# gongaa/video-layout-generation

Measured on AMD Instinct MI355X. Metric: training clips/sec at (B,T,N)=(32,16,64) d=256; 1/2/4/8-GPU scaling, higher is better.
Workload: dtype f32

## Files before the change

include/vlg_hip.h:

```cpp
#ifndef VLG_HIP_H
#define VLG_HIP_H

#include <stdint.h>

typedef uint16_t vlg_bf16;

#ifdef __cplusplus
extern "C" {
#endif

#define VLG_ERR_SHAPE   1001
#define VLG_ERR_ALIGN   1002

int         vlg_abi_version(void);
const char* vlg_build_arch(void);

#ifdef VLG_DIAG
void vlg_debug_set_clock_probe(unsigned long long* buf);
void vlg_debug_set_conv_probe(unsigned long long* buf);
void vlg_debug_set_gemm_bk(int bk);
void vlg_debug_set_gemm_run(int run);
#endif

int vlg_embed_fwd(const int64_t* slot_class, const float* slot_box,
                  const float* cls_emb, const float* box_w, const float* box_b,
                  const float* time_emb, float* x,
                  int B, int T, int N, int d, int vocab, void* stream);
int vlg_embed_bwd_slabs(void);
int vlg_embed_bwd_slabs_for(int B, int T, int N, int d, int vocab);
int vlg_embed_bwd(const float* dx, const int64_t* slot_class, const float* slot_box,
                  float* slabs, int64_t slab_stride, int64_t slab_capacity,
                  int B, int T, int N, int d, int vocab, void* stream);

int vlg_layernorm_fwd(const float* x, const float* gamma, const float* beta,
                      float* y, float* mean, float* rstd,
                      int64_t rows, int d, float eps, void* stream);
int vlg_layernorm_fwd_bf16(const float* x, const float* gamma, const float* beta,
                           vlg_bf16* y, float* mean, float* rstd,
                           int64_t rows, int d, float eps, void* stream);
int vlg_layernorm_bwd_slabs(int64_t rows);
int vlg_layernorm_bwd(const float* dy, const float* x, const float* mean, const float* rstd,
                      const float* gamma, const float* dres, float* dx_out,
                      float* slabs, int64_t slab_stride, int64_t slab_capacity,
                      int64_t rows, int d, void* stream);
int vlg_layernorm_bwd_bf16(const vlg_bf16* dy, const float* x, const float* mean, const float* rstd,
                           const float* gamma, const float* dres, float* dx_out,
                           float* slabs, int64_t slab_stride, int64_t slab_capacity,
                           int64_t rows, int d, void* stream);

#define VLG_EPI_NONE   0
#define VLG_EPI_BIAS   1
#define VLG_EPI_GELU   2
#define VLG_EPI_RESID  4
#define VLG_EPI_DGELU  8
#define VLG_EPI_BF16   16
#define VLG_EPI_SPLIT3 256
#define VLG_EPI_ACT_GELU 512
#define VLG_EPI_GELU_GRAD 1024
#define VLG_EPI_MUL    2048
#define VLG_EPI_A_BF16   32
#define VLG_EPI_B_BF16   64
#define VLG_EPI_OUT_BF16 128
int vlg_linear_fwd(const void* A, int lda, const void* W, int ldw, const float* bias,
                   void* C, int ldc, const void* aux_in, void* aux_out,
                   int64_t M, int N, int K, int epilogue, void* stream);
int vlg_linear_dgrad(const void* dY, int ldy, const void* W, int ldw,
                     void* dX, int ldx, const void* aux_in,
                     int64_t M, int N, int K, int epilogue, void* stream);
int vlg_linear_wgrad_slabs(int64_t M, int N, int K);
int vlg_linear_wgrad_slabs_for(int64_t M, int N, int K, int flags);
int vlg_linear_wgrad(const void* dY, int ldy, const void* X, int ldx,
                     float* slabs, int64_t slab_stride, int64_t slab_capacity,
                     int64_t M, int N, int K, int flags , void* stream);
int vlg_linear_dgrad_wgrad(const void* dY, int ldy, const void* W, int ldw, void* dX, int ldx, const void* aux_in,
                           const void* X, int ldxx, float* slabs, int64_t slab_stride, int64_t slab_capacity,
                           int64_t M, int N, int K, int epilogue,
                           const int64_t* rider_table , int rider_rows, void* stream);
#define VLG_CALL_FWD   0
#define VLG_CALL_DGRAD 1
#define VLG_CALL_WGRAD 2
#define VLG_CALL_PAIR  3
#define VLG_GEMM_F32   0
#define VLG_GEMM_BF16  1
#define VLG_GEMM_F32X3 2
typedef struct vlg_gemm_problem {
    int bm, bn, bk;
    int run;
    int splits;
    int blocks;
    int64_t rows_per_split;
} vlg_gemm_problem;
typedef struct vlg_gemm_plan {
    int family;
    int launches;
    int problems;
    int fused;
    vlg_gemm_problem p[2];
} vlg_gemm_plan;
int vlg_linear_plan(int call, int64_t M, int N, int K, int flags, int lda, int ldb, int ldc, int ldxx, vlg_gemm_plan* plan);


int vlg_attention_fwd(const float* qkv, float* o, int64_t n_seq, int T, int d, void* stream);
int vlg_attention_bwd(const float* qkv, const float* dout, float* dqkv,
                      int64_t n_seq, int T, int d, void* stream);
int vlg_attention_fwd_bf16(const vlg_bf16* qkv, vlg_bf16* o, int64_t n_seq, int T, int d, void* stream);
int vlg_attention_bwd_bf16(const vlg_bf16* qkv, const vlg_bf16* dout, vlg_bf16* dqkv,
                           int64_t n_seq, int T, int d, void* stream);

int vlg_layout_loss_scratch(void);
int vlg_layout_loss(const float* out, int ld, const int64_t* tgt_class, const float* tgt_box,
                    const float* valid, float* dout, float* loss_out, float* scratch,
                    int B, int T, int N, int n_classes, float beta, float iou_eps,
                    float w_reg, float w_iou, float w_ce, void* stream);

int vlg_attention_clip_fwd(const float* qkv, const float* valid, float* out, float* lse,
                           int64_t B, int T, int N, int d, void* stream);
int vlg_attention_clip_bwd(const float* qkv, const float* valid, const float* out, const float* dout, const float* lse,
                           float* delta, float* dqkv, int64_t B, int T, int N, int d, void* stream);
int vlg_attention_clip_fwd_bf16(const vlg_bf16* qkv, const float* valid, vlg_bf16* out, float* lse,
                                int64_t B, int T, int N, int d, void* stream);
int vlg_attention_clip_bwd_bf16(const vlg_bf16* qkv, const float* valid, const vlg_bf16* out, const vlg_bf16* dout,
                                const float* lse, float* delta, vlg_bf16* dqkv,
                                int64_t B, int T, int N, int d, void* stream);

int vlg_reduce_slabs(const float* slabs, int64_t slab_stride, int n_slabs,
                     float* dst, int64_t len, void* stream);

int vlg_adam_step_graph(float* param, const float* grad, float* exp_avg, float* exp_avg_sq, vlg_bf16* shadow,
                        int64_t n, float* state, int advance, float lr, float beta1, float beta2, float eps,
                        float grad_scale, void* stream);

int vlg_reduce_slabs_table(const int64_t* table, int n_rows, int blocks_per_row, void* stream);
int vlg_sum_partials_table(const int64_t* table, int n_rows, void* stream);

int vlg_adam_step(float* param, const float* grad, float* exp_avg, float* exp_avg_sq,
                  int64_t n, int step, float lr, float beta1, float beta2, float eps,
                  float grad_scale, void* stream);
int vlg_adam_step_bf16(float* param, const float* grad, float* exp_avg, float* exp_avg_sq, vlg_bf16* shadow,
                       int64_t n, int step, float lr, float beta1, float beta2, float eps,
                       float grad_scale, void* stream);

int vlg_image_loss_scratch(void);
int vlg_ce_nchw(const float* logits, const int64_t* target, float* dlogits, float* loss,
                float* scratch, int b, int C, int64_t hw, float grad_scale, void* stream);
int vlg_l1_mean(const float* a, const float* b, float* da, float* loss, float* scratch,
                int64_t n, float grad_scale, void* stream);
int vlg_gradient_loss(const float* a, const float* b, float* da, float* loss, float* scratch,
                      int planes, int H, int W, float grad_scale, void* stream);
int vlg_ssim_loss(const float* x, const float* y, float* dx, float* loss, float* scratch,
                  int b, int C, int H, int W, float grad_scale, void* stream);
int vlg_affine_nchw(const float* src, float* dst, int b, int C, int64_t hw, const float* shift_host,
                    const float* scale_host, void* stream);
int vlg_prep_input(const float* e1, const float* seg1, const float* frame1,
                   const float* frame2, const float* seg2, const float* e2,
                   const float* frame3, const int64_t* seg3,
                   float* x10, float* frame3_out, int64_t* seg3_out,
                   int b, int H, int W, int flip, void* stream);

int vlg_argmax_nchw(const float* logits, float* out, int b, int C, int64_t hw, void* stream);
int vlg_rollout_input(const float* e_a, const float* seg_a, const float* img_a, const float* img_b,
                      const float* seg_b, const float* e_b, float* x10, int b, int64_t hw, void* stream);

#define VLG_CEPI_BIAS   1
#define VLG_CEPI_RESID  2
#define VLG_CEPI_PRELU  4
#define VLG_CEPI_DPRELU 8
#define VLG_CEPI_ACCUM  16
#define VLG_CEPI_CIN4   32
int vlg_conv3x3_fwd(const float* in, const float* w, const float* bias, float* out, const float* resid,
                    const float* rowmask, const float* prelu_slope, const int* rowtab, int64_t rows_out,
                    int cin_p, int cout, int cout_p, int wp_in, int act_ch, int epilogue,
                    float* workspace ,
                    int64_t workspace_capacity , void* stream);
int vlg_conv3x3_fwd_splits(int64_t rows_out, int cin_p, int cout, int cout_p);
int64_t vlg_conv3x3_fwd_workspace(int64_t rows_out, int cin_p, int cout, int cout_p);
int vlg_conv3x3_dgrad_slabs(int64_t rows_in, int cin_p);
int vlg_conv3x3_dgrad(const float* dout, const float* w, float* din, const float* x_in,
                      const float* rowmask_in, const float* prelu_slope, float* da_slab,
                      const int* tap_tables, int64_t tab_stride, int64_t rows_in, int cin_p, int cout_p,
                      int wp, int act_ch, int epilogue,
                      float* workspace ,
                      int64_t workspace_capacity ,
                      int da_capacity , void* stream);
int vlg_conv3x3_dgrad_splits(int64_t rows_in, int cin_p, int cout_p);
int64_t vlg_conv3x3_dgrad_workspace(int64_t rows_in, int cin_p, int cout_p);
int vlg_conv3x3_wgrad_slabs(int64_t rows, int cin_p, int cout_p);
int vlg_conv3x3_wgrad(const float* dout, const float* in, float* slabs, int64_t slab_stride, int64_t slab_capacity,
                      const int* rowtab, const float* prelu_slope, int64_t rows, int cin_p, int cout_p,
                      int wp_in, int act_ch, void* stream);
int vlg_conv3x3_fwd_bf16(const float* in, const float* w, const float* bias, float* out, const float* resid,
                         const float* rowmask, const float* prelu_slope, const int* rowtab, int64_t rows_out,
                         int cin_p, int cout, int cout_p, int wp_in, int act_ch, int epilogue, float* workspace,
                         int64_t workspace_capacity, void* stream);
int vlg_conv3x3_fwd_bf16_splits(int64_t rows_out, int cin_p, int cout, int cout_p);
int64_t vlg_conv3x3_fwd_bf16_workspace(int64_t rows_out, int cin_p, int cout, int cout_p);
int vlg_conv3x3_dgrad_bf16_slabs(int64_t rows_in, int cin_p);
int vlg_conv3x3_dgrad_bf16(const float* dout, const float* w, float* din, const float* x_in,
                           const float* rowmask_in, const float* prelu_slope, float* da_slab,
                           const int* tap_tables, int64_t tab_stride, int64_t rows_in, int cin_p, int cout_p,
                           int wp, int act_ch, int epilogue, float* workspace, int64_t workspace_capacity,
                           int da_capacity, void* stream);
int vlg_conv3x3_dgrad_bf16_splits(int64_t rows_in, int cin_p, int cout_p);
int64_t vlg_conv3x3_dgrad_bf16_workspace(int64_t rows_in, int cin_p, int cout_p);
int vlg_conv3x3_wgrad_bf16_slabs(int64_t rows, int cin_p, int cout_p);
int vlg_conv3x3_wgrad_bf16(const float* dout, const float* in, float* slabs, int64_t slab_stride, int64_t slab_capacity,
                           const int* rowtab, const float* prelu_slope, int64_t rows, int cin_p, int cout_p,
                           int wp_in, int act_ch, void* stream);
int vlg_nchw_to_padded(const float* src, float* dst, int b, int C, int H, int W, int cp, int coord_c0, void* stream);
int vlg_padded_to_nchw(const float* src, float* dst, int b, int C, int H, int W, int cp, void* stream);
int vlg_fill_coords(float* dst, int b, int H, int W, int cp, int coord_c0, void* stream);
int vlg_upsample2x_fwd(const float* in, float* out, int b, int h, int w, int cp, void* stream);
int vlg_upsample2x_bwd(const float* dout, float* din, int b, int h, int w, int cp, int accumulate, void* stream);
int vlg_maxpool2x2(const float* in, float* out, int b, int h, int w, int cp, void* stream);
int vlg_score1x1_relu(const float* in, const float* w, const float* bias, float* out, int b, int H, int W,
                      int C, int cp, void* stream);
int vlg_hed_head(const float* s0, const float* s1, const float* s2, const float* s3, const float* s4,
                 const float* combine_w, const float* combine_b, float* out , int b, int H, int W,
                 void* stream);
int vlg_maxpool2x2_bwd(const float* in, const float* dout, float* din, int b, int h, int w, int cp, void* stream);
int vlg_l1_relu_padded(const float* a, const float* b, float* da, float* loss, float* scratch ,
                       int64_t rows, int cp, int64_t count, float grad_scale, void* stream);
int vlg_add_rows(float* dst, const float* src, int64_t n, int accumulate, void* stream);
int vlg_sum_partials(const float* partials, int n, float* dst, int accumulate, void* stream);

#ifdef __cplusplus
}
#endif
#endif
```

video-layout-generation_amd/csrc/layernorm.hip:

```cpp
#include "common.h"

#define LN_BLOCK 256
#define LN_WAVES (LN_BLOCK / 64)
#define LN_BWD_MAX_BLOCKS 512

template <int E, bool V4>
struct RowIO {
    template <typename EL>
    __device__ static __forceinline__ void load(const EL* __restrict__ row, int lane, float (&v)[E]) {
        if constexpr (V4) {
#pragma unroll
            for (int i = 0; i < E / 4; ++i) {
                const float4 t = ld4(row + 4 * lane + 256 * i);
                v[4 * i] = t.x; v[4 * i + 1] = t.y; v[4 * i + 2] = t.z; v[4 * i + 3] = t.w;
            }
        } else {
#pragma unroll
            for (int i = 0; i < E; ++i) v[i] = ld1(row + lane + 64 * i);
        }
    }
    template <typename EL>
    __device__ static __forceinline__ void store(EL* __restrict__ row, int lane, const float (&v)[E]) {
        if constexpr (V4) {
#pragma unroll
            for (int i = 0; i < E / 4; ++i)
                st4(row + 4 * lane + 256 * i, make_float4(v[4 * i], v[4 * i + 1], v[4 * i + 2], v[4 * i + 3]));
        } else {
#pragma unroll
            for (int i = 0; i < E; ++i) st1(row + lane + 64 * i, v[i]);
        }
    }
    __device__ static __forceinline__ int col(int lane, int j) {
        if constexpr (V4) return 4 * lane + 256 * (j >> 2) + (j & 3);
        else return lane + 64 * j;
    }
};

#define LN_ROWS(E) ((E) <= 4 ? 4 : (E) <= 8 ? 2 : 1)

template <int E, bool V4, typename EY = float>
__global__ __launch_bounds__(LN_BLOCK) void ln_fwd_kernel(
    const float* __restrict__ x, const float* __restrict__ gamma, const float* __restrict__ beta,
    EY* __restrict__ y, float* __restrict__ mean, float* __restrict__ rstd, int64_t rows, float eps) {
    constexpr int d = E * 64, R = LN_ROWS(E);
    const int lane = threadIdx.x & 63;
    const int64_t wave = (int64_t)blockIdx.x * LN_WAVES + (threadIdx.x >> 6);
    const int64_t nwaves = (int64_t)gridDim.x * LN_WAVES;
    float g[E], b[E];
    RowIO<E, V4>::load(gamma, lane, g);
    RowIO<E, V4>::load(beta, lane, b);
    for (int64_t r0 = wave * R; r0 < rows; r0 += nwaves * R) {
        float v[R][E];
#pragma unroll
        for (int i = 0; i < R; ++i) {
            const int64_t r = r0 + i < rows ? r0 + i : rows - 1;
            RowIO<E, V4>::load(x + r * d, lane, v[i]);
        }
#pragma unroll
        for (int i = 0; i < R; ++i) {
            float s = 0.f;
#pragma unroll
            for (int j = 0; j < E; ++j) s += v[i][j];
            const float mu = wave_sum(s) * (1.0f / d);
            float q = 0.f;
#pragma unroll
            for (int j = 0; j < E; ++j) { const float t = v[i][j] - mu; q += t * t; }
            const float rs = 1.0f / sqrtf(wave_sum(q) * (1.0f / d) + eps);
#pragma unroll
            for (int j = 0; j < E; ++j) v[i][j] = (v[i][j] - mu) * rs * g[j] + b[j];
            if (r0 + i < rows) {
                RowIO<E, V4>::store(y + (r0 + i) * d, lane, v[i]);
                if (lane == 0) { mean[r0 + i] = mu; rstd[r0 + i] = rs; }
            }
        }
    }
}

template <int E, bool V4, typename EY = float>
__global__ __launch_bounds__(LN_BLOCK) void ln_bwd_kernel(
    const EY* __restrict__ dy, const float* __restrict__ x, const float* __restrict__ mean,
    const float* __restrict__ rstd, const float* __restrict__ gamma, const float* __restrict__ dres,
    float* __restrict__ dx_out, float* __restrict__ slabs, int64_t slab_stride, int64_t rows) {
    constexpr int d = E * 64, R = LN_ROWS(E);
    __shared__ float red[LN_WAVES][2 * d];
    const int lane = threadIdx.x & 63, w = threadIdx.x >> 6;
    const int64_t wave = (int64_t)blockIdx.x * LN_WAVES + w;
    const int64_t nwaves = (int64_t)gridDim.x * LN_WAVES;
    float g[E], dg[E], db[E];
    RowIO<E, V4>::load(gamma, lane, g);
#pragma unroll
    for (int j = 0; j < E; ++j) { dg[j] = 0.f; db[j] = 0.f; }
    for (int64_t r0 = wave * R; r0 < rows; r0 += nwaves * R) {
        float gy[R][E], xv[R][E], o[R][E], mu[R], rs[R];
#pragma unroll
        for (int i = 0; i < R; ++i) {
            const int64_t r = r0 + i < rows ? r0 + i : rows - 1;
            RowIO<E, V4>::load(dy + r * d, lane, gy[i]);
            RowIO<E, V4>::load(x + r * d, lane, xv[i]);
            if (dres != nullptr) RowIO<E, V4>::load(dres + r * d, lane, o[i]);
            else {
#pragma unroll
                for (int j = 0; j < E; ++j) o[i][j] = 0.f;
            }
            mu[i] = mean[r];
            rs[i] = rstd[r];
        }
#pragma unroll
        for (int i = 0; i < R; ++i) {
            const float live = r0 + i < rows ? 1.f : 0.f;
            float s1 = 0.f, s2 = 0.f;
#pragma unroll
            for (int j = 0; j < E; ++j) {
                const float xh = (xv[i][j] - mu[i]) * rs[i];
                const float gl = gy[i][j] * live;
                const float a = gy[i][j] * g[j];
                dg[j] += gl * xh;
                db[j] += gl;
                s1 += a;
                s2 += a * xh;
                xv[i][j] = xh;
                gy[i][j] = a;
            }
            s1 = wave_sum(s1) * (1.0f / d);
            s2 = wave_sum(s2) * (1.0f / d);
#pragma unroll
            for (int j = 0; j < E; ++j) o[i][j] += rs[i] * (gy[i][j] - s1 - xv[i][j] * s2);
            if (r0 + i < rows) RowIO<E, V4>::store(dx_out + (r0 + i) * d, lane, o[i]);
        }
    }
#pragma unroll
    for (int j = 0; j < E; ++j) {
        const int c = RowIO<E, V4>::col(lane, j);
        red[w][c] = dg[j];
        red[w][d + c] = db[j];
    }
    __syncthreads();
    float* slab = slabs + (int64_t)blockIdx.x * slab_stride;
    for (int c = threadIdx.x; c < 2 * d; c += LN_BLOCK) {
        float s = 0.f;
#pragma unroll
        for (int k = 0; k < LN_WAVES; ++k) s += red[k][c];
        slab[c] = s;
    }
}

static int ln_fwd_blocks(int64_t rows) {
    int64_t b = (rows + LN_WAVES - 1) / LN_WAVES;
    return (int)(b > 2048 ? 2048 : (b < 1 ? 1 : b));
}
static int ln_bwd_blocks(int64_t rows) {
    int64_t b = (rows + LN_WAVES - 1) / LN_WAVES;
    return (int)(b > LN_BWD_MAX_BLOCKS ? LN_BWD_MAX_BLOCKS : (b < 1 ? 1 : b));
}

#define LN_DISPATCH(d, CALL)                                 \
    switch (d) {                                             \
        case 64:   { CALL(1, false) } break;                 \
        case 128:  { CALL(2, false) } break;                 \
        case 192:  { CALL(3, false) } break;                 \
        case 256:  { CALL(4, true) } break;                  \
        case 512:  { CALL(8, true) } break;                  \
        case 768:  { CALL(12, true) } break;                 \
        case 1024: { CALL(16, true) } break;                 \
        default: return VLG_ERR_SHAPE;                       \
    }

extern "C" int vlg_layernorm_fwd(const float* x, const float* gamma, const float* beta, float* y,
                                 float* mean, float* rstd, int64_t rows, int d, float eps, void* stream) {
    if (rows < 1) return VLG_ERR_SHAPE;
    if (!vlg_aligned16(x) || !vlg_aligned16(y) || !vlg_aligned16(gamma) || !vlg_aligned16(beta)) return VLG_ERR_ALIGN;
    const dim3 grid(ln_fwd_blocks(rows)), block(LN_BLOCK);
    hipStream_t s = (hipStream_t)stream;
#define CALL(E, V4) hipLaunchKernelGGL((ln_fwd_kernel<E, V4>), grid, block, 0, s, x, gamma, beta, y, mean, rstd, rows, eps);
    LN_DISPATCH(d, CALL)
#undef CALL
    return vlg_last_error();
}

extern "C" int vlg_layernorm_bwd_slabs(int64_t rows) { return ln_bwd_blocks(rows); }

extern "C" int vlg_layernorm_bwd(const float* dy, const float* x, const float* mean, const float* rstd,
                                 const float* gamma, const float* dres, float* dx_out, float* slabs,
                                 int64_t slab_stride, int64_t slab_capacity, int64_t rows, int d, void* stream) {
    if (rows < 1 || slab_stride < 2 * (int64_t)d) return VLG_ERR_SHAPE;
    if (slab_capacity < (int64_t)ln_bwd_blocks(rows) * slab_stride) return VLG_ERR_SHAPE;
    if (!vlg_aligned16(dy) || !vlg_aligned16(x) || !vlg_aligned16(gamma) || !vlg_aligned16(dx_out) ||
        (dres && !vlg_aligned16(dres))) return VLG_ERR_ALIGN;
    const dim3 grid(ln_bwd_blocks(rows)), block(LN_BLOCK);
    hipStream_t s = (hipStream_t)stream;
#define CALL(E, V4) hipLaunchKernelGGL((ln_bwd_kernel<E, V4>), grid, block, 0, s, dy, x, mean, rstd, gamma, dres, dx_out, slabs, slab_stride, rows);
    LN_DISPATCH(d, CALL)
#undef CALL
    return vlg_last_error();
}

extern "C" int vlg_layernorm_fwd_bf16(const float* x, const float* gamma, const float* beta, vlg_bf16* y,
                                      float* mean, float* rstd, int64_t rows, int d, float eps, void* stream) {
    if (rows < 1) return VLG_ERR_SHAPE;
    if (!vlg_aligned16(x) || !vlg_aligned8(y) || !vlg_aligned16(gamma) || !vlg_aligned16(beta)) return VLG_ERR_ALIGN;
    const dim3 grid(ln_fwd_blocks(rows)), block(LN_BLOCK);
    hipStream_t s = (hipStream_t)stream;
    bf16_t* yb = reinterpret_cast<bf16_t*>(y);
#define CALL(E, V4) hipLaunchKernelGGL((ln_fwd_kernel<E, V4, bf16_t>), grid, block, 0, s, x, gamma, beta, yb, mean, rstd, rows, eps);
    LN_DISPATCH(d, CALL)
#undef CALL
    return vlg_last_error();
}

extern "C" int vlg_layernorm_bwd_bf16(const vlg_bf16* dy, const float* x, const float* mean, const float* rstd,
                                      const float* gamma, const float* dres, float* dx_out, float* slabs,
                                      int64_t slab_stride, int64_t slab_capacity, int64_t rows, int d, void* stream) {
    if (rows < 1 || slab_stride < 2 * (int64_t)d) return VLG_ERR_SHAPE;
    if (slab_capacity < (int64_t)ln_bwd_blocks(rows) * slab_stride) return VLG_ERR_SHAPE;
    if (!vlg_aligned8(dy) || !vlg_aligned16(x) || !vlg_aligned16(gamma) || !vlg_aligned16(dx_out) ||
        (dres && !vlg_aligned16(dres))) return VLG_ERR_ALIGN;
    const dim3 grid(ln_bwd_blocks(rows)), block(LN_BLOCK);
    hipStream_t s = (hipStream_t)stream;
    const bf16_t* dyb = reinterpret_cast<const bf16_t*>(dy);
#define CALL(E, V4) hipLaunchKernelGGL((ln_bwd_kernel<E, V4, bf16_t>), grid, block, 0, s, dyb, x, mean, rstd, gamma, dres, dx_out, slabs, slab_stride, rows);
    LN_DISPATCH(d, CALL)
#undef CALL
    return vlg_last_error();
}
```

video-layout-generation_amd/csrc/loss.hip:

```cpp
#include "common.h"

#define LOSS_BLOCK 256
#define LOSS_TOK 128
#define LOSS_ROWF 28
#define LOSS_MAX_BLOCKS 1024
#define NCLS 20
#define NOUT (NCLS + 4)
#define LOSS_F4 (NOUT / 4)
#define LOSS_NV (LOSS_TOK * LOSS_F4 / LOSS_BLOCK)

#define LOSS_SCRATCH (4 + 4 * LOSS_MAX_BLOCKS)

__global__ __launch_bounds__(LOSS_BLOCK) void layout_loss_kernel(
    const float* __restrict__ out, int ld, const int64_t* __restrict__ tgt_class,
    const float* __restrict__ tgt_box, const float* __restrict__ valid, float* __restrict__ dout,
    float* __restrict__ scratch, float* __restrict__ loss_out, int B, int T, int N, float beta, float iou_eps,
    float w_reg, float w_iou, float w_ce) {
    __shared__ __attribute__((aligned(16))) float rows[LOSS_TOK * LOSS_ROWF];
    __shared__ float red[LOSS_BLOCK / 64];
    __shared__ float cnt_sh;
    __shared__ int last_sh;
    const int64_t M = (int64_t)B * T * N;
    const int tid = threadIdx.x;
    float inv_cnt = 0.f;
    float s_reg = 0.f, s_iou = 0.f, s_ce = 0.f;
    for (int64_t m0 = (int64_t)blockIdx.x * LOSS_TOK; m0 < M; m0 += (int64_t)gridDim.x * LOSS_TOK) {
        float4 stage[LOSS_NV];
#pragma unroll
        for (int i = 0; i < LOSS_NV; ++i) {
            const int f = tid + i * LOSS_BLOCK, tok = f / LOSS_F4, c = f - tok * LOSS_F4;
            stage[i] = (m0 + tok < M) ? ld4(out + (m0 + tok) * ld + 4 * c) : f4_zero();
        }
        const int64_t m = m0 + tid;
        const bool mine = tid < LOSS_TOK && m < M;
        float w = 0.f;
        int64_t cls = 0;
        float4 tb = f4_zero();
        if (mine) {
            const int t = (int)(m % T);
            const int64_t bn = m / T;
            const int n = (int)(bn % N);
            const int64_t b = bn / N;
            const int64_t src = (b * T + t) * N + n;
            w = valid[src];
            cls = tgt_class[src];
            tb = ld4(tgt_box + src * 4);
        }
        if (m0 == (int64_t)blockIdx.x * LOSS_TOK) {
            float c = 0.f;
            const int64_t n4 = M >> 2;
            int64_t i = tid;
            for (; i + 15 * LOSS_BLOCK < n4; i += 16 * LOSS_BLOCK) {
                float4 v[16];
#pragma unroll
                for (int u = 0; u < 16; ++u) v[u] = ld4(valid + 4 * (i + u * LOSS_BLOCK));
#pragma unroll
                for (int u = 0; u < 16; ++u) c += (v[u].x + v[u].y) + (v[u].z + v[u].w);
            }
            for (; i < n4; i += LOSS_BLOCK) {
                const float4 v = ld4(valid + 4 * i);
                c += (v.x + v.y) + (v.z + v.w);
            }
            for (int64_t j = 4 * n4 + tid; j < M; j += LOSS_BLOCK) c += valid[j];
            c = block_sum(c, red);
            if (tid == 0) cnt_sh = 1.0f / fmaxf(c, 1.0f);
            __syncthreads();
            inv_cnt = cnt_sh;
        }
#pragma unroll
        for (int i = 0; i < LOSS_NV; ++i) {
            const int f = tid + i * LOSS_BLOCK, tok = f / LOSS_F4, c = f - tok * LOSS_F4;
            st4(rows + tok * LOSS_ROWF + 4 * c, stage[i]);
        }
        __syncthreads();
        if (mine) {
            float* row = rows + tid * LOSS_ROWF;
            float v[NOUT];
#pragma unroll
            for (int c = 0; c < LOSS_F4; ++c) {
                const float4 q = ld4(row + 4 * c);
                v[4 * c] = q.x; v[4 * c + 1] = q.y; v[4 * c + 2] = q.z; v[4 * c + 3] = q.w;
            }
            float g[NOUT];
            cls = cls < 0 ? 0 : (cls >= NCLS ? NCLS - 1 : cls);
            float mx = v[0];
#pragma unroll
            for (int c = 1; c < NCLS; ++c) mx = fmaxf(mx, v[c]);
            float se = 0.f, vt = 0.f;
#pragma unroll
            for (int c = 0; c < NCLS; ++c) {
                g[c] = expf(v[c] - mx);
                se += g[c];
                vt = (c == cls) ? v[c] : vt;
            }
            const float ce = logf(se) + mx - vt;
            const float gs = w * inv_cnt * w_ce / se;
#pragma unroll
            for (int c = 0; c < NCLS; ++c) g[c] = g[c] * gs - ((c == cls) ? w * inv_cnt * w_ce : 0.f);
            const float tg[4] = {tb.x, tb.y, tb.z, tb.w};
            float p[4], dp[4];
            float reg = 0.f;
#pragma unroll
            for (int k = 0; k < 4; ++k) {
                p[k] = 1.0f / (1.0f + expf(-v[NCLS + k]));
                const float df = p[k] - tg[k], ad = fabsf(df);
                const bool quad = ad < beta;
                reg += quad ? 0.5f * df * df / beta : ad - 0.5f * beta;
                dp[k] = (quad ? df / beta : (df > 0.f ? 1.f : (df < 0.f ? -1.f : 0.f))) * (w_reg * 0.25f);
            }
            const float ax1 = p[0] - 0.5f * p[2], ax2 = p[0] + 0.5f * p[2];
            const float ay1 = p[1] - 0.5f * p[3], ay2 = p[1] + 0.5f * p[3];
            const float bx1 = tg[0] - 0.5f * tg[2], bx2 = tg[0] + 0.5f * tg[2];
            const float by1 = tg[1] - 0.5f * tg[3], by2 = tg[1] + 0.5f * tg[3];
            const float iw_raw = fminf(ax2, bx2) - fmaxf(ax1, bx1);
            const float ih_raw = fminf(ay2, by2) - fmaxf(ay1, by1);
            const float iw = fmaxf(iw_raw, 0.f), ih = fmaxf(ih_raw, 0.f);
            const float inter = iw * ih;
            const float uni = p[2] * p[3] + tg[2] * tg[3] - inter;
            const float den = uni + iou_eps;
            const float iou = inter / den;
            const float di_dinter = (den + inter) / (den * den);
            const float di_darea = -inter / (den * den);
            const float x2s = (ax2 < bx2) ? 1.f : (ax2 == bx2 ? 0.5f : 0.f);
            const float x1s = (ax1 > bx1) ? 1.f : (ax1 == bx1 ? 0.5f : 0.f);
            const float y2s = (ay2 < by2) ? 1.f : (ay2 == by2 ? 0.5f : 0.f);
            const float y1s = (ay1 > by1) ? 1.f : (ay1 == by1 ? 0.5f : 0.f);
            const float diw = (iw_raw >= 0.f) ? ih * di_dinter : 0.f;
            const float dih = (ih_raw >= 0.f) ? iw * di_dinter : 0.f;
            float di[4];
            di[0] = diw * (x2s - x1s);
            di[1] = dih * (y2s - y1s);
            di[2] = diw * 0.5f * (x2s + x1s) + di_darea * p[3];
            di[3] = dih * 0.5f * (y2s + y1s) + di_darea * p[2];
#pragma unroll
            for (int k = 0; k < 4; ++k)
                g[NCLS + k] = (dp[k] - w_iou * di[k]) * p[k] * (1.f - p[k]) * w * inv_cnt;
#pragma unroll
            for (int c = 0; c < LOSS_F4; ++c)
                st4(row + 4 * c, make_float4(g[4 * c], g[4 * c + 1], g[4 * c + 2], g[4 * c + 3]));
            s_reg += w * reg * 0.25f;
            s_iou += w * (1.f - iou);
            s_ce += w * ce;
        }
        __syncthreads();
#pragma unroll
        for (int i = 0; i < LOSS_NV; ++i) {
            const int f = tid + i * LOSS_BLOCK, tok = f / LOSS_F4, c = f - tok * LOSS_F4;
            if (m0 + tok < M) st4(dout + (m0 + tok) * ld + 4 * c, ld4(rows + tok * LOSS_ROWF + 4 * c));
        }
        __syncthreads();
    }
    s_reg = block_sum(s_reg, red);
    s_iou = block_sum(s_iou, red);
    s_ce = block_sum(s_ce, red);
    if (tid == 0) {
        float* part = scratch + 4 + 4 * blockIdx.x;
        part[0] = s_reg * inv_cnt; part[1] = s_iou * inv_cnt; part[2] = s_ce * inv_cnt; part[3] = 0.f;
        __threadfence();
        int* ticket = reinterpret_cast<int*>(scratch) + 1;
        const int drawn = atomicAdd(ticket, 1);
        last_sh = (drawn == (int)gridDim.x - 1) ? 1 : 0;
    }
    __syncthreads();
    if (last_sh && tid < 64) {
        __threadfence();
        float a = 0.f, b = 0.f, c = 0.f;
        for (int i = tid; i < (int)gridDim.x; i += 64) {
            const float4 q = ld4(scratch + 4 + 4 * i);
            a += q.x; b += q.y; c += q.z;
        }
        a = wave_sum(a); b = wave_sum(b); c = wave_sum(c);
        if (tid == 0) {
            loss_out[0] = w_reg * a + w_iou * b + w_ce * c;
            loss_out[1] = a; loss_out[2] = b; loss_out[3] = c;
            *(reinterpret_cast<int*>(scratch) + 1) = 0;
        }
    }
}

extern "C" int vlg_layout_loss_scratch(void) { return LOSS_SCRATCH; }

extern "C" int vlg_layout_loss(const float* out, int ld, const int64_t* tgt_class, const float* tgt_box,
                               const float* valid, float* dout, float* loss_out, float* scratch, int B, int T,
                               int N, int n_classes, float beta, float iou_eps, float w_reg, float w_iou,
                               float w_ce, void* stream) {
    if (n_classes != NCLS || B < 1 || T < 1 || N < 1 || ld < NOUT || (ld & 3) || !(beta > 0.f)) return VLG_ERR_SHAPE;
    if (!vlg_aligned16(out) || !vlg_aligned16(dout) || !vlg_aligned16(tgt_box) || !vlg_aligned16(valid)) return VLG_ERR_ALIGN;
    const int64_t M = (int64_t)B * T * N;
    if (!loss_out || !scratch || !vlg_aligned16(scratch)) return VLG_ERR_ALIGN;
    int64_t blocks = (M + LOSS_TOK - 1) / LOSS_TOK;
    if (blocks > LOSS_MAX_BLOCKS) blocks = LOSS_MAX_BLOCKS;
    hipStream_t s = (hipStream_t)stream;
    hipLaunchKernelGGL(layout_loss_kernel, dim3((unsigned)blocks), dim3(LOSS_BLOCK), 0, s, out, ld, tgt_class,
                       tgt_box, valid, dout, scratch, loss_out, B, T, N, beta, iou_eps, w_reg, w_iou, w_ce);
    return vlg_last_error();
}
```

video-layout-generation_amd/vlg/engine.py:

```python
from __future__ import annotations

import math
import os
from typing import Dict, Optional

import torch

from . import hip
from .hip import (EPI_A_BF16, EPI_B_BF16, EPI_BIAS, EPI_DGELU, EPI_GELU, EPI_NONE, EPI_OUT_BF16, EPI_RESID,
                  call, ptr)
from .spec import (ADAM_BETA1, ADAM_BETA2, ADAM_EPS, ADAM_LR, BOX_DIM, IOU_EPS, LN_EPS, LOSS_W_CE,
                   LOSS_W_REG, LOSS_W_STRUCT, SMOOTH_L1_BETA, LayoutConfig, param_layout)


def init_params(cfg: LayoutConfig, seed: int) -> Dict[str, torch.Tensor]:
    layout, _ = param_layout(cfg)
    g = torch.Generator().manual_seed(seed)
    fan_in = {name[:-2] + "_b": shape[1] for name, (_, shape) in layout.items() if name.endswith("_w")}
    out: Dict[str, torch.Tensor] = {}
    for name, (_, shape) in layout.items():
        base = name.split(".")[-1]
        if base in ("cls_emb", "time_emb"):
            t = torch.randn(shape, generator=g, dtype=torch.float32)
        elif base.endswith("_g"):
            t = torch.ones(shape)
        elif base.startswith("ln") and base.endswith("_b"):
            t = torch.zeros(shape)
        elif base.endswith("_w"):
            t = (torch.rand(shape, generator=g, dtype=torch.float32) * 2 - 1) * (1.0 / math.sqrt(shape[1]))
        else:
            t = (torch.rand(shape, generator=g, dtype=torch.float32) * 2 - 1) * (1.0 / math.sqrt(fan_in[name]))
        out[name] = t
    return out


class LayoutEngine:

    def __init__(self, cfg: LayoutConfig, device: torch.device, seed: int = 1024,
                 lr: float = ADAM_LR, beta1: float = ADAM_BETA1, precision: str = "fp32", padded_slots: bool = True):
        cfg.validate()
        if precision not in ("fp32", "bf16", "bf16_mfma", "fp32x3"):
            raise ValueError("precision must be fp32, fp32x3, bf16 or bf16_mfma")
        self.padded_slots = bool(padded_slots)
        self._masked = self.padded_slots
        self.precision = precision
        self.gemm_flags = {"fp32": 0, "fp32x3": hip.EPI_SPLIT3}.get(precision, hip.EPI_BF16)
        self.bf16_store = precision == "bf16"
        self.gelu_grad_saved = precision in ("fp32", "bf16", "bf16_mfma") and os.environ.get("VLG_GELU_GRAD_SAVED", "1") != "0"
        self._epi_ff1 = EPI_BIAS | EPI_GELU | (hip.EPI_GELU_GRAD if self.gelu_grad_saved else 0)
        self._epi_dff2 = hip.EPI_MUL if self.gelu_grad_saved else EPI_DGELU
        self._sfx = "_bf16" if self.bf16_store else ""
        hip.load()
        if device.type != "cuda":
            raise hip.HipError("LayoutEngine needs a HIP device (got %s); there is no CPU path" % device)
        self.cfg, self.device = cfg, device
        self.lr, self.beta1 = float(lr), float(beta1)
        self.layout, self.n_params = param_layout(cfg)
        f32 = dict(dtype=torch.float32, device=device)
        self.params = torch.zeros(self.n_params, **f32)
        self.grads_ext = torch.zeros(self.n_params + 4, **f32)
        self.grads = self.grads_ext[:self.n_params]
        self.exp_avg = torch.zeros(self.n_params, **f32)
        self.exp_avg_sq = torch.zeros(self.n_params, **f32)
        self.step_count = 0
        self.adam_state = None
        self.params_bf16 = torch.zeros(self.n_params, dtype=torch.bfloat16, device=device) if self.bf16_store else None
        self.load_params(init_params(cfg, seed))
        self._alloc_workspace(cfg.tokens)
        self.loss_out = self.grads_ext[self.n_params:]
        self.timer = None

    def view(self, flat: torch.Tensor, name: str) -> torch.Tensor:
        off, shape = self.layout[name]
        return flat[off:off + math.prod(shape)].view(shape)

    def p(self, name: str) -> torch.Tensor:
        return self.view(self.params, name)

    def pw(self, name: str) -> torch.Tensor:
        return self.view(self.params_bf16 if self.bf16_store else self.params, name)

    def _sync_device_step(self) -> None:
        if self.adam_state is not None:
            self.adam_state.view(torch.int32)[2] = int(self.step_count)

    def _refresh_shadow(self) -> None:
        if self.params_bf16 is not None:
            self.params_bf16.copy_(self.params)

    def g(self, name: str) -> torch.Tensor:
        return self.view(self.grads, name)

    def load_params(self, tensors: Dict[str, torch.Tensor]) -> None:
        for name in self.layout:
            self.p(name).copy_(tensors[name].to(torch.float32))
        self._refresh_shadow()

    def named_params(self) -> Dict[str, torch.Tensor]:
        return {n: self.p(n) for n in self.layout}

    def named_grads(self) -> Dict[str, torch.Tensor]:
        return {n: self.g(n) for n in self.layout}

    def state_dict(self) -> Dict[str, object]:
        return {"params": self.params.detach().cpu().clone(), "exp_avg": self.exp_avg.cpu().clone(),
                "exp_avg_sq": self.exp_avg_sq.cpu().clone(), "step": self.step_count,
                "layout": {k: (o, tuple(s)) for k, (o, s) in self.layout.items()}}

    def load_state_dict(self, sd: Dict[str, object]) -> None:
        if tuple(sd["params"].shape) != (self.n_params,):
            raise ValueError("checkpoint has %d parameters, model has %d" % (sd["params"].numel(), self.n_params))
        self.params.copy_(sd["params"])
        self._refresh_shadow()
        self.exp_avg.copy_(sd["exp_avg"])
        self.exp_avg_sq.copy_(sd["exp_avg_sq"])
        self.step_count = int(sd["step"])
        self._sync_device_step()

    def optimizer_state(self) -> Dict[str, object]:
        return {"exp_avg": self.exp_avg.cpu().clone(), "exp_avg_sq": self.exp_avg_sq.cpu().clone(),
                "step": int(self.step_count), "lr": self.lr, "beta1": self.beta1}

    def load_optimizer(self, st: Dict[str, object]) -> None:
        if st["exp_avg"].numel() != self.n_params:
            raise ValueError("optimizer state has %d elements, model has %d" % (st["exp_avg"].numel(), self.n_params))
        self.exp_avg.copy_(st["exp_avg"])
        self.exp_avg_sq.copy_(st["exp_avg_sq"])
        self.step_count = int(st["step"])
        self._sync_device_step()

    def _alloc_workspace(self, tokens: int) -> None:
        cfg, d, ff = self.cfg, self.cfg.d, self.cfg.d_ff
        f32 = dict(dtype=torch.float32, device=self.device)
        M = self.capacity = tokens
        L = cfg.n_layers
        lib = hip.load()
        act = dict(dtype=torch.bfloat16 if self.bf16_store else torch.float32, device=self.device)
        self.x = torch.empty(L + 1, M, d, **f32)
        self.h1 = torch.empty(L, M, d, **act)
        self.qkv = torch.empty(L, M, 3 * d, **act)
        self.att = torch.empty(L, M, d, **act)
        self.xmid = torch.empty(L, M, d, **f32)
        self.h2 = torch.empty(L, M, d, **act)
        self.u = torch.empty(L, M, ff, **act)
        self.gl = torch.empty(L, M, ff, **act)
        self.stats = torch.empty(2 * L + 1, 2, M, **f32)
        self.xf = torch.empty(M, d, **act)
        self.out = torch.empty(M, cfg.n_out, **f32)
        self.dout = torch.empty(M, cfg.n_out, **f32)
        self.dx = torch.empty(M, d, **f32)
        self.dh = torch.empty(M, d, **act)
        self.du = torch.empty(M, ff, **act)
        self.dqkv = torch.empty(M, 3 * d, **act)
        self.loss_scratch = torch.zeros(lib.vlg_layout_loss_scratch(), **f32)
        if cfg.attention == "clip":
            self.lse = torch.empty(L, cfg.n_heads * M, **f32)
            self.delta = torch.empty(cfg.n_heads * M, **f32)
        emb_len = self.layout["l0.ln1_g"][0]
        need = [lib.vlg_embed_bwd_slabs() * emb_len, lib.vlg_layernorm_bwd_slabs(M) * 2 * d]
        for (n, k) in ((3 * d, d), (d, d), (ff, d), (d, ff), (cfg.n_out, d)):
            need.append(lib.vlg_linear_wgrad_slabs_for(M, n, k, self.gemm_flags) * (n * k + n))
        self.side = torch.cuda.Stream(device=self.device)
        self.overlap_wgrad = os.environ.get("VLG_OVERLAP_WGRAD", "0") == "1"
        self.group_reduce = not self.overlap_wgrad
        self.pair_backward = (not self.overlap_wgrad and self.precision in ("fp32", "bf16")
                              and os.environ.get("VLG_PAIR_BACKWARD", "1") == "1")
        self.ride_reduces = False
        if self.group_reduce:
            pad = lambda v: (v + 3) // 4 * 4
            layer = sum(pad(v) for v in need[2:6]) + 2 * pad(need[1])
            head = pad(need[6]) + pad(need[1])
            self.garenas = [torch.empty(max(layer, head, pad(need[0])), **f32) for _ in range(2)]
            self._gsel = 0
            self._goff = 0
            self._grows: list = []
            self._gtables: Dict[tuple, torch.Tensor] = {}
            self._pending = None
            self.ride_reduces = self.pair_backward and os.environ.get("VLG_RIDE_REDUCE", "1") == "1"
        else:
            self.slabs = torch.empty(max(need[:2]), **f32)
            self.slabs_w = torch.empty(max(need[2:]), **f32)

    @staticmethod
    def _stream() -> int:
        return torch.cuda.current_stream().cuda_stream

    def _arena(self, kind: str, need: int = 0) -> torch.Tensor:
        if self.group_reduce:
            garena = self.garenas[self._gsel]
            off = self._goff
            if off + need > garena.numel():
                raise RuntimeError("partial-sum arena of %d floats is too small for %d more" % (garena.numel(), need))
            self._goff = off + (need + 3) // 4 * 4
            self._gcur = garena.data_ptr() + 4 * off
            return garena[off:off + need]
        return self.slabs_w if kind == "w" else self.slabs

    def _reduce(self, kind: str, stride: int, n_slabs: int, dst_off: int, dst_len: int) -> None:
        dst = self.grads.data_ptr() + 4 * dst_off
        if self.group_reduce:
            self._grows.append((self._gcur, stride, n_slabs, dst, dst_len))
            return
        call("vlg_reduce_slabs", ptr(self.slabs_w if kind == "w" else self.slabs), stride, n_slabs, dst, dst_len, self._stream())

    def _table(self, rows: tuple) -> torch.Tensor:
        table = self._gtables.get(rows)
        if table is None:
            table = torch.tensor([v for row in rows for v in row], dtype=torch.int64, device=self.device)
            self._gtables[rows] = table
        return table

    def _join_reduces(self, defer: bool = False, then=None) -> None:
        if not self.group_reduce:
            if then is not None:
                then()
            return
        rows = tuple(self._grows)
        self._grows = []
        self._goff = 0
        if defer and self.ride_reduces and rows and self._pending is None:
            self._pending = (rows, then)
            self._gsel ^= 1
            return
        waiting, self._pending = self._pending, None
        if waiting is not None:
            rows = waiting[0] + rows
        if rows:
            call("vlg_reduce_slabs_table", ptr(self._table(rows)), len(rows), 128, self._stream())
        if waiting is not None and waiting[1] is not None:
            waiting[1]()
        if then is not None:
            then()

    def _take_rider(self):
        if not self.group_reduce or self._pending is None:
            self._rider_bytes = 0.0
            return 0, 0, None
        (rows, then), self._pending = self._pending, None
        self._rider_bytes = 4.0 * sum((n_slabs + 1) * length for (_, _, n_slabs, _, length) in rows)
        return ptr(self._table(rows)), len(rows), then

    def _timed(self, family: str, flops: float, name: str, *args, nbytes: float = 0.0) -> None:
        if self.timer is None or (self.timer.only is not None and family not in self.timer.only):
            call(name, *args)
        else:
            with self.timer.section(family, flops, nbytes):
                call(name, *args)

    @staticmethod
    def _storage_bits(a=None, b=None, out=None) -> int:
        bf = torch.bfloat16
        return ((EPI_A_BF16 if a is not None and a.dtype == bf else 0) | (EPI_B_BF16 if b is not None and b.dtype == bf else 0) |
                (EPI_OUT_BF16 if out is not None and out.dtype == bf else 0))

    def _linear(self, a, w, b, c, M, N, K, epi, aux_in=None, aux_out=None):
        nb = (a.element_size() * M * K + w.element_size() * N * K +
              c.element_size() * M * N * (1 + (aux_in is not None) + (aux_out is not None)))
        flags = epi | self.gemm_flags | self._storage_bits(a, w, c)
        self._timed("gemm_fwd" if N > 32 else "gemm_head", 2.0 * M * N * K, "vlg_linear_fwd", ptr(a), K, ptr(w), K,
                    ptr(b), ptr(c), N, ptr(aux_in), ptr(aux_out), M, N, K, flags, self._stream(), nbytes=nb)

    def _dgrad(self, dy, w, dx, M, N, K, epi=EPI_NONE, aux_in=None):
        nb = dy.element_size() * M * N + w.element_size() * N * K + dx.element_size() * M * K * (1 + (aux_in is not None))
        flags = epi | self.gemm_flags | self._storage_bits(dy, w, dx)
        self._timed("gemm_dgrad", 2.0 * M * N * K, "vlg_linear_dgrad", ptr(dy), N, ptr(w), K, ptr(dx), K,
                    ptr(aux_in), M, N, K, flags, self._stream(), nbytes=nb)

    def _wgrad(self, dy, x, wname, M, N, K):
        lib = hip.load()
        stride = N * K + N
        flags = self.gemm_flags | self._storage_bits(dy, x)
        n_slabs = lib.vlg_linear_wgrad_slabs_for(M, N, K, flags)
        arena = self._arena("w", n_slabs * stride)
        s = self._stream()
        self._timed("gemm_wgrad" if N > 32 else "gemm_head", 2.0 * M * N * K, "vlg_linear_wgrad", ptr(dy), N, ptr(x),
                    K, ptr(arena), stride, arena.numel(), M, N, K, flags, s,
                    nbytes=dy.element_size() * M * N + x.element_size() * M * K + 4.0 * n_slabs * stride)
        self._reduce("w", stride, n_slabs, self.layout[wname][0], stride)

    def _dgrad_wgrad(self, dy, w, dx, x, wname, M, N, K, epi=EPI_NONE, aux_in=None):
        lib = hip.load()
        stride = N * K + N
        n_slabs = lib.vlg_linear_wgrad_slabs_for(M, N, K, self.gemm_flags)
        arena = self._arena("w", n_slabs * stride)
        nb = (dy.element_size() * M * N * 2 + w.element_size() * N * K + dx.element_size() * M * K * (1 + (aux_in is not None)) +
              x.element_size() * M * K + 4.0 * n_slabs * stride)
        bits = self._storage_bits(dy, w, dx)
        if (x.dtype == torch.bfloat16) != (w.dtype == torch.bfloat16):
            raise ValueError("paired backward: X and W must have the same storage type")
        rider, rider_rows, then = self._take_rider()
        self._timed("gemm_pair", 4.0 * M * N * K, "vlg_linear_dgrad_wgrad", ptr(dy), N, ptr(w), K, ptr(dx), K, ptr(aux_in),
                    ptr(x), K, ptr(arena), stride, arena.numel(), M, N, K, epi | self.gemm_flags | bits, rider, rider_rows,
                    self._stream(), nbytes=nb + self._rider_bytes)
        if then is not None:
            then()
        self._reduce("w", stride, n_slabs, self.layout[wname][0], stride)

    def _attn_fwd(self, l: int, batch, B, T, N, M) -> None:
        d, s = self.cfg.d, self._stream()
        if self.cfg.attention == "clip":
            fl = 4.0 * B * d * N * N * T * (T + 1) / 2.0
            e = self.qkv.element_size()
            self._timed("attn_clip_fwd", fl, "vlg_attention_clip_fwd" + self._sfx, ptr(self.qkv[l]),
                        ptr(batch["valid"]) if self._masked else 0, ptr(self.att[l]), ptr(self.lse[l]), B, T, N, d, s,
                        nbytes=4.0 * e * M * d)
            return
        self._timed("attn_fwd", 0.0, "vlg_attention_fwd" + self._sfx, ptr(self.qkv[l]), ptr(self.att[l]), B * N, T, d, s,
                    nbytes=4.0 * self.qkv.element_size() * M * d)

    def _attn_bwd(self, l: int, batch, B, T, N, M) -> None:
        d, s = self.cfg.d, self._stream()
        if self.cfg.attention == "clip":
            fl = 2.5 * 4.0 * B * d * N * N * T * (T + 1) / 2.0
            e = self.qkv.element_size()
            self._timed("attn_clip_bwd", fl, "vlg_attention_clip_bwd" + self._sfx, ptr(self.qkv[l]),
                        ptr(batch["valid"]) if self._masked else 0, ptr(self.att[l]), ptr(self.dh), ptr(self.lse[l]),
                        ptr(self.delta), ptr(self.dqkv), B, T, N, d, s, nbytes=7.0 * e * M * d)
            return
        self._timed("attn_bwd", 0.0, "vlg_attention_bwd" + self._sfx, ptr(self.qkv[l]), ptr(self.dh), ptr(self.dqkv), B * N, T, d, s,
                    nbytes=7.0 * self.qkv.element_size() * M * d)

    def _ln_fwd(self, x, gname, y, stat, M):
        d = self.cfg.d
        self._timed("ln_fwd", 0.0, "vlg_layernorm_fwd_bf16" if y.dtype == torch.bfloat16 else "vlg_layernorm_fwd", ptr(x), ptr(self.p(gname)),
                    ptr(self.p(gname[:-1] + "b")), ptr(y), ptr(stat[0]), ptr(stat[1]), M, d, LN_EPS, self._stream(),
                    nbytes=(4.0 + y.element_size()) * M * d)

    def _ln_bwd(self, dy, x, stat, gname, dres, dx_out, M):
        d = self.cfg.d
        lib = hip.load()
        n_slabs = lib.vlg_layernorm_bwd_slabs(M)
        arena = self._arena("s", n_slabs * 2 * d)
        s = self._stream()
        self._timed("ln_bwd", 0.0, "vlg_layernorm_bwd_bf16" if dy.dtype == torch.bfloat16 else "vlg_layernorm_bwd", ptr(dy), ptr(x), ptr(stat[0]),
                    ptr(stat[1]), ptr(self.p(gname)), ptr(dres), ptr(dx_out), ptr(arena), 2 * d, arena.numel(), M, d, s,
                    nbytes=(dy.element_size() + 4.0 + 4.0 + (4.0 if dres is not None else 0.0)) * M * d)
        self._reduce("s", 2 * d, n_slabs, self.layout[gname][0], 2 * d)

    def _check_batch(self, batch) -> tuple:
        sc = batch["slot_class"]
        B, T, N = sc.shape
        if T != self.cfg.T:
            raise ValueError("batch has T=%d, engine was built for T=%d" % (T, self.cfg.T))
        M = B * T * N
        if M > self.capacity:
            raise ValueError("batch of %d tokens exceeds workspace capacity %d" % (M, self.capacity))
        for k, dt in (("slot_class", torch.int64), ("slot_box", torch.float32), ("tgt_class", torch.int64),
                      ("tgt_box", torch.float32), ("valid", torch.float32)):
            t = batch[k]
            if t.dtype != dt or not t.is_cuda or not t.is_contiguous():
                raise ValueError("batch[%r] must be a contiguous %s HIP tensor" % (k, dt))
        return B, T, N, M

    def forward(self, batch: Dict[str, torch.Tensor], padded_slots: Optional[bool] = None) -> torch.Tensor:
        cfg, d, ff = self.cfg, self.cfg.d, self.cfg.d_ff
        B, T, N, M = self._check_batch(batch)
        self._masked = self.padded_slots if padded_slots is None else bool(padded_slots)
        self._shape = (B, T, N, M)
        s = self._stream()
        self._timed("embed_fwd", 0.0, "vlg_embed_fwd", ptr(batch["slot_class"]), ptr(batch["slot_box"]), ptr(self.p("cls_emb")),
                    ptr(self.p("box_w")), ptr(self.p("box_b")), ptr(self.p("time_emb")), ptr(self.x[0]),
                    B, T, N, d, cfg.vocab, s, nbytes=4.0 * M * d + 24.0 * M)
        for l in range(cfg.n_layers):
            pre = "l%d." % l
            x = self.x[l]
            self._ln_fwd(x, pre + "ln1_g", self.h1[l], self.stats[2 * l], M)
            self._linear(self.h1[l], self.pw(pre + "qkv_w"), self.p(pre + "qkv_b"), self.qkv[l], M, 3 * d, d, EPI_BIAS)
            self._attn_fwd(l, batch, B, T, N, M)
            self._linear(self.att[l], self.pw(pre + "proj_w"), self.p(pre + "proj_b"), self.xmid[l], M, d, d,
                         EPI_BIAS | EPI_RESID, aux_in=x)
            self._ln_fwd(self.xmid[l], pre + "ln2_g", self.h2[l], self.stats[2 * l + 1], M)
            self._linear(self.h2[l], self.pw(pre + "ff1_w"), self.p(pre + "ff1_b"), self.gl[l], M, ff, d,
                         self._epi_ff1, aux_out=self.u[l])
            self._linear(self.gl[l], self.pw(pre + "ff2_w"), self.p(pre + "ff2_b"), self.x[l + 1], M, d, ff,
                         EPI_BIAS | EPI_RESID, aux_in=self.xmid[l])
        L = cfg.n_layers
        self._ln_fwd(self.x[L], "lnf_g", self.xf, self.stats[2 * L], M)
        self._linear(self.xf, self.pw("head_w"), self.p("head_b"), self.out, M, cfg.n_out, d, EPI_BIAS)
        self._timed("loss", 0.0, "vlg_layout_loss", ptr(self.out), cfg.n_out, ptr(batch["tgt_class"]), ptr(batch["tgt_box"]),
                    ptr(batch["valid"]), ptr(self.dout), ptr(self.loss_out), ptr(self.loss_scratch), B, T, N,
                    cfg.n_classes, SMOOTH_L1_BETA, IOU_EPS, LOSS_W_REG, LOSS_W_STRUCT, LOSS_W_CE, s,
                    nbytes=(2.0 * 4 * cfg.n_out + 8 + 16 + 4) * M)
        return self.loss_out

    def backward(self, batch: Dict[str, torch.Tensor], reducer=None) -> None:
        cfg, d, ff = self.cfg, self.cfg.d, self.cfg.d_ff
        B, T, N, M = self._shape
        main = torch.cuda.current_stream(self.device)
        side = self.side if self.overlap_wgrad else main
        s = main.cuda_stream
        L = cfg.n_layers
        last_read: Dict[str, torch.cuda.Event] = {}

        def on_side(reads, fn):
            if side is main:
                fn()
                return
            e = torch.cuda.Event()
            e.record(main)
            side.wait_event(e)
            with torch.cuda.stream(side):
                fn()
                done = torch.cuda.Event()
                done.record(side)
            for name in reads:
                last_read[name] = done

        def before_write(*names):
            for name in names:
                e = last_read.pop(name, None)
                if e is not None:
                    main.wait_event(e)

        def join():
            if side is not main:
                e = torch.cuda.Event()
                e.record(side)
                main.wait_event(e)
                last_read.clear()

        if self.group_reduce:
            self._gsel, self._goff, self._grows, self._pending = 0, 0, [], None
        on_side(("dout",), lambda: self._wgrad(self.dout, self.xf, "head_w", M, cfg.n_out, d))
        self._dgrad(self.dout, self.pw("head_w"), self.dh, M, cfg.n_out, d)
        self._ln_bwd(self.dh, self.x[L], self.stats[2 * L], "lnf_g", None, self.dx, M)
        ready = (lambda tag: (lambda: reducer.ready(tag))) if reducer is not None else (lambda tag: None)
        if reducer is not None or self.group_reduce:
            join()
            self._join_reduces(defer=self.pair_backward, then=ready("head"))
        for l in reversed(range(L)):
            pre = "l%d." % l
            if self.pair_backward:
                self._dgrad_wgrad(self.dx, self.pw(pre + "ff2_w"), self.du, self.gl[l], pre + "ff2_w", M, d, ff, self._epi_dff2, aux_in=self.u[l])
                self._dgrad_wgrad(self.du, self.pw(pre + "ff1_w"), self.dh, self.h2[l], pre + "ff1_w", M, ff, d)
                self._ln_bwd(self.dh, self.xmid[l], self.stats[2 * l + 1], pre + "ln2_g", self.dx, self.dx, M)
                self._dgrad_wgrad(self.dx, self.pw(pre + "proj_w"), self.dh, self.att[l], pre + "proj_w", M, d, d)
                self._attn_bwd(l, batch, B, T, N, M)
                self._dgrad_wgrad(self.dqkv, self.pw(pre + "qkv_w"), self.dh, self.h1[l], pre + "qkv_w", M, 3 * d, d)
                self._ln_bwd(self.dh, self.x[l], self.stats[2 * l], pre + "ln1_g", self.dx, self.dx, M)
                self._join_reduces(defer=True, then=ready("l%d" % l))
                continue
            on_side(("dx",), lambda: self._wgrad(self.dx, self.gl[l], pre + "ff2_w", M, d, ff))
            before_write("du")
            self._dgrad(self.dx, self.pw(pre + "ff2_w"), self.du, M, d, ff, self._epi_dff2, aux_in=self.u[l])
            on_side(("du",), lambda: self._wgrad(self.du, self.h2[l], pre + "ff1_w", M, ff, d))
            self._dgrad(self.du, self.pw(pre + "ff1_w"), self.dh, M, ff, d)
            before_write("dx")
            self._ln_bwd(self.dh, self.xmid[l], self.stats[2 * l + 1], pre + "ln2_g", self.dx, self.dx, M)
            on_side(("dx",), lambda: self._wgrad(self.dx, self.att[l], pre + "proj_w", M, d, d))
            self._dgrad(self.dx, self.pw(pre + "proj_w"), self.dh, M, d, d)
            before_write("dqkv")
            self._attn_bwd(l, batch, B, T, N, M)
            on_side(("dqkv",), lambda: self._wgrad(self.dqkv, self.h1[l], pre + "qkv_w", M, 3 * d, d))
            self._dgrad(self.dqkv, self.pw(pre + "qkv_w"), self.dh, M, 3 * d, d)
            before_write("dx")
            self._ln_bwd(self.dh, self.x[l], self.stats[2 * l], pre + "ln1_g", self.dx, self.dx, M)
            if reducer is not None or self.group_reduce:
                join()
                self._join_reduces()
            if reducer is not None:
                reducer.ready("l%d" % l)
        join()
        self._backward_tail(batch, B, T, N, M, reducer)

    def _backward_tail(self, batch, B, T, N, M, reducer) -> None:
        cfg, d = self.cfg, self.cfg.d
        lib = hip.load()
        s = self._stream()
        emb_len = self.layout["l0.ln1_g"][0]
        n_slabs = lib.vlg_embed_bwd_slabs_for(B, T, N, d, cfg.vocab)
        arena = self._arena("s", n_slabs * emb_len)
        self._timed("embed_bwd", 0.0, "vlg_embed_bwd", ptr(self.dx), ptr(batch["slot_class"]), ptr(batch["slot_box"]), ptr(arena),
                    emb_len, arena.numel(), B, T, N, d, cfg.vocab, s, nbytes=4.0 * M * d + 24.0 * M)
        self._reduce("s", emb_len, n_slabs, 0, emb_len)
        self._join_reduces(then=(lambda: reducer.ready("embed")) if reducer is not None else None)

    def forward_backward(self, batch: Dict[str, torch.Tensor], reducer=None) -> torch.Tensor:
        loss = self.forward(batch)
        self.backward(batch, reducer)
        return loss

    def train_step(self, batch: Dict[str, torch.Tensor], reducer=None) -> torch.Tensor:
        loss = self.forward_backward(batch, reducer)
        if reducer is not None:
            split = self.layout["l0.ln1_g"][0]
            reducer.wait(keep=("embed",))
            self.adam_step(reducer.grad_scale, lo=split, hi=self.n_params)
            reducer.wait()
            self.adam_step(reducer.grad_scale, lo=0, hi=split, advance=False)
        else:
            self.adam_step()
        return loss

    def adam_step(self, grad_scale: float = 1.0, lo: int = 0, hi: Optional[int] = None, advance: bool = True) -> None:
        hi = self.n_params if hi is None else hi
        if advance:
            self.step_count += 1
        o = 4 * lo
        shadow = self.params_bf16.data_ptr() + o // 2 if self.params_bf16 is not None else 0
        if self.adam_state is not None:
            call("vlg_adam_step_graph", self.params.data_ptr() + o, self.grads.data_ptr() + o, self.exp_avg.data_ptr() + o,
                 self.exp_avg_sq.data_ptr() + o, shadow, hi - lo, ptr(self.adam_state), 1 if advance else 0, self.lr,
                 self.beta1, ADAM_BETA2, ADAM_EPS, grad_scale, self._stream())
            return
        if self.params_bf16 is not None:
            call("vlg_adam_step_bf16", self.params.data_ptr() + o, self.grads.data_ptr() + o, self.exp_avg.data_ptr() + o,
                 self.exp_avg_sq.data_ptr() + o, shadow, hi - lo, self.step_count, self.lr,
                 self.beta1, ADAM_BETA2, ADAM_EPS, grad_scale, self._stream())
            return
        self._timed("adam", 0.0, "vlg_adam_step", self.params.data_ptr() + o, self.grads.data_ptr() + o, self.exp_avg.data_ptr() + o,
                    self.exp_avg_sq.data_ptr() + o, hi - lo, self.step_count, self.lr, self.beta1, ADAM_BETA2, ADAM_EPS,
                    grad_scale, self._stream(), nbytes=28.0 * (hi - lo))

    def use_device_step_counter(self) -> None:
        if self.adam_state is None:
            st = torch.zeros(4, dtype=torch.float32, device=self.device)
            st.view(torch.int32)[2] = int(self.step_count)
            self.adam_state = st

    def capture_train_step(self, example_batch: Dict[str, torch.Tensor]):
        self._check_batch(example_batch)
        self.use_device_step_counter()
        static = {k: example_batch[k].clone() for k in ("slot_class", "slot_box", "tgt_class", "tgt_box", "valid")}
        side = torch.cuda.Stream(device=self.device)
        side.wait_stream(torch.cuda.current_stream(self.device))
        keep = (self.params.clone(), self.exp_avg.clone(), self.exp_avg_sq.clone(), self.adam_state.clone(), self.step_count)
        with torch.cuda.stream(side):
            self.train_step(static)
        torch.cuda.current_stream(self.device).wait_stream(side)
        torch.cuda.synchronize(self.device)
        self.params.copy_(keep[0]); self.exp_avg.copy_(keep[1]); self.exp_avg_sq.copy_(keep[2])
        self.adam_state.copy_(keep[3]); self.step_count = keep[4]
        self._refresh_shadow()
        timer, self.timer = self.timer, None
        graph = torch.cuda.CUDAGraph()
        with torch.cuda.graph(graph, stream=side):
            self.train_step(static)
        self.timer = timer
        self.params.copy_(keep[0]); self.exp_avg.copy_(keep[1]); self.exp_avg_sq.copy_(keep[2])
        self.adam_state.copy_(keep[3]); self.step_count = keep[4]
        self._refresh_shadow()

        def run(batch: Dict[str, torch.Tensor]) -> torch.Tensor:
            for k, t in static.items():
                if batch[k] is not t:
                    t.copy_(batch[k], non_blocking=True)
            graph.replay()
            self.step_count += 1
            return self.loss_out
        run.graph, run.static_batch = graph, static
        return run

    def outputs_btn(self) -> tuple:
        B, T, N, M = self._shape
        o = self.out[:M].view(B, N, T, self.cfg.n_out).permute(0, 2, 1, 3)
        return o[..., :self.cfg.n_classes], o[..., self.cfg.n_classes:]


class KernelTimer:

    def __init__(self, only=None):
        self.records = {}
        self.only = only

    class _Section:
        def __init__(self, timer, family, flops, nbytes=0.0):
            self.t, self.family, self.flops, self.nbytes = timer, family, flops, nbytes

        def __enter__(self):
            self.s = torch.cuda.Event(enable_timing=True)
            self.e = torch.cuda.Event(enable_timing=True)
            self.s.record()

        def __exit__(self, *a):
            self.e.record()
            self.t.records.setdefault(self.family, []).append((self.s, self.e, self.flops, self.nbytes))

    def section(self, family: str, flops: float, nbytes: float = 0.0):
        return KernelTimer._Section(self, family, flops, nbytes)

    def summary(self):
        out = {}
        for fam, recs in self.records.items():
            ms = [s.elapsed_time(e) for s, e, _, _ in recs]
            fl = [f for _, _, f, _ in recs]
            nb = [b for _, _, _, b in recs]
            out[fam] = {"launches": len(ms), "avg_ms": sum(ms) / len(ms), "total_ms": sum(ms),
                        "flops_per_launch": sum(fl) / len(fl), "bytes_per_launch": sum(nb) / len(nb)}
        return out
```

video-layout-generation_amd/vlg/hip.py:

```python
from __future__ import annotations

import ctypes
import os
from ctypes import c_char_p, c_float, c_int, c_int64, c_void_p

_HERE = os.path.dirname(os.path.abspath(__file__))
LIB_PATH = os.environ.get("VLG_HIP_LIB") or os.path.join(os.path.dirname(_HERE), "libvlg_hip.so")

EPI_NONE, EPI_BIAS, EPI_GELU, EPI_RESID, EPI_DGELU, EPI_BF16 = 0, 1, 2, 4, 8, 16
EPI_A_BF16, EPI_B_BF16, EPI_OUT_BF16, EPI_SPLIT3 = 32, 64, 128, 256
EPI_ACT_GELU = 512
EPI_GELU_GRAD, EPI_MUL = 1024, 2048

P, I, L, F = c_void_p, c_int, c_int64, c_float

SIGNATURES = {
    "vlg_abi_version": (I, []),
    "vlg_build_arch": (c_char_p, []),
    "vlg_embed_fwd": (I, [P, P, P, P, P, P, P, I, I, I, I, I, P]),
    "vlg_embed_bwd_slabs": (I, []),
    "vlg_embed_bwd_slabs_for": (I, [I, I, I, I, I]),
    "vlg_embed_bwd": (I, [P, P, P, P, L, L, I, I, I, I, I, P]),
    "vlg_layernorm_fwd": (I, [P, P, P, P, P, P, L, I, F, P]),
    "vlg_layernorm_fwd_bf16": (I, [P, P, P, P, P, P, L, I, F, P]),
    "vlg_layernorm_bwd_slabs": (I, [L]),
    "vlg_layernorm_bwd": (I, [P, P, P, P, P, P, P, P, L, L, L, I, P]),
    "vlg_layernorm_bwd_bf16": (I, [P, P, P, P, P, P, P, P, L, L, L, I, P]),
    "vlg_linear_fwd": (I, [P, I, P, I, P, P, I, P, P, L, I, I, I, P]),
    "vlg_linear_dgrad": (I, [P, I, P, I, P, I, P, L, I, I, I, P]),
    "vlg_linear_wgrad_slabs": (I, [L, I, I]),
    "vlg_linear_dgrad_wgrad": (I, [P, I, P, I, P, I, P, P, I, P, L, L, L, I, I, I, P, I, P]),
    "vlg_linear_wgrad_slabs_for": (I, [L, I, I, I]),
    "vlg_linear_wgrad": (I, [P, I, P, I, P, L, L, L, I, I, I, P]),
    "vlg_linear_plan": (I, [I, L, I, I, I, I, I, I, I, P]),
    "vlg_attention_fwd": (I, [P, P, L, I, I, P]),
    "vlg_attention_bwd": (I, [P, P, P, L, I, I, P]),
    "vlg_attention_fwd_bf16": (I, [P, P, L, I, I, P]),
    "vlg_attention_bwd_bf16": (I, [P, P, P, L, I, I, P]),
    "vlg_attention_clip_fwd": (I, [P, P, P, P, L, I, I, I, P]),
    "vlg_attention_clip_bwd": (I, [P, P, P, P, P, P, P, L, I, I, I, P]),
    "vlg_attention_clip_fwd_bf16": (I, [P, P, P, P, L, I, I, I, P]),
    "vlg_attention_clip_bwd_bf16": (I, [P, P, P, P, P, P, P, L, I, I, I, P]),
    "vlg_layout_loss_scratch": (I, []),
    "vlg_layout_loss": (I, [P, I, P, P, P, P, P, P, I, I, I, I, F, F, F, F, F, P]),
    "vlg_reduce_slabs": (I, [P, L, I, P, L, P]),
    "vlg_reduce_slabs_table": (I, [P, I, I, P]),
    "vlg_sum_partials_table": (I, [P, I, P]),
    "vlg_adam_step": (I, [P, P, P, P, L, I, F, F, F, F, F, P]),
    "vlg_adam_step_graph": (I, [P, P, P, P, P, L, P, I, F, F, F, F, F, P]),
    "vlg_adam_step_bf16": (I, [P, P, P, P, P, L, I, F, F, F, F, F, P]),
    "vlg_image_loss_scratch": (I, []),
    "vlg_ce_nchw": (I, [P, P, P, P, P, I, I, L, F, P]),
    "vlg_l1_mean": (I, [P, P, P, P, P, L, F, P]),
    "vlg_gradient_loss": (I, [P, P, P, P, P, I, I, I, F, P]),
    "vlg_ssim_loss": (I, [P, P, P, P, P, I, I, I, I, F, P]),
    "vlg_affine_nchw": (I, [P, P, I, I, L, P, P, P]),
    "vlg_prep_input": (I, [P, P, P, P, P, P, P, P, P, P, P, I, I, I, I, P]),
    "vlg_argmax_nchw": (I, [P, P, I, I, L, P]),
    "vlg_rollout_input": (I, [P, P, P, P, P, P, P, I, L, P]),
    "vlg_conv3x3_fwd": (I, [P, P, P, P, P, P, P, P, L, I, I, I, I, I, I, P, L, P]),
    "vlg_conv3x3_fwd_splits": (I, [L, I, I, I]),
    "vlg_conv3x3_fwd_workspace": (L, [L, I, I, I]),
    "vlg_conv3x3_dgrad_slabs": (I, [L, I]),
    "vlg_conv3x3_dgrad": (I, [P, P, P, P, P, P, P, P, L, L, I, I, I, I, I, P, L, I, P]),
    "vlg_conv3x3_dgrad_splits": (I, [L, I, I]),
    "vlg_conv3x3_dgrad_workspace": (L, [L, I, I]),
    "vlg_conv3x3_wgrad_slabs": (I, [L, I, I]),
    "vlg_conv3x3_wgrad": (I, [P, P, P, L, L, P, P, L, I, I, I, I, P]),
    "vlg_conv3x3_fwd_bf16": (I, [P, P, P, P, P, P, P, P, L, I, I, I, I, I, I, P, L, P]),
    "vlg_conv3x3_fwd_bf16_splits": (I, [L, I, I, I]),
    "vlg_conv3x3_fwd_bf16_workspace": (L, [L, I, I, I]),
    "vlg_conv3x3_dgrad_bf16_slabs": (I, [L, I]),
    "vlg_conv3x3_dgrad_bf16": (I, [P, P, P, P, P, P, P, P, L, L, I, I, I, I, I, P, L, I, P]),
    "vlg_conv3x3_dgrad_bf16_splits": (I, [L, I, I]),
    "vlg_conv3x3_dgrad_bf16_workspace": (L, [L, I, I]),
    "vlg_conv3x3_wgrad_bf16_slabs": (I, [L, I, I]),
    "vlg_conv3x3_wgrad_bf16": (I, [P, P, P, L, L, P, P, L, I, I, I, I, P]),
    "vlg_nchw_to_padded": (I, [P, P, I, I, I, I, I, I, P]),
    "vlg_padded_to_nchw": (I, [P, P, I, I, I, I, I, P]),
    "vlg_fill_coords": (I, [P, I, I, I, I, I, P]),
    "vlg_upsample2x_fwd": (I, [P, P, I, I, I, I, P]),
    "vlg_upsample2x_bwd": (I, [P, P, I, I, I, I, I, P]),
    "vlg_maxpool2x2": (I, [P, P, I, I, I, I, P]),
    "vlg_score1x1_relu": (I, [P, P, P, P, I, I, I, I, I, P]),
    "vlg_hed_head": (I, [P, P, P, P, P, P, P, P, I, I, I, P]),
    "vlg_maxpool2x2_bwd": (I, [P, P, P, I, I, I, I, P]),
    "vlg_l1_relu_padded": (I, [P, P, P, P, P, L, I, L, F, P]),
    "vlg_add_rows": (I, [P, P, L, I, P]),
    "vlg_sum_partials": (I, [P, I, P, I, P]),
}
DIAG_SIGNATURES = {
    "vlg_debug_set_clock_probe": (None, [P]),
    "vlg_debug_set_conv_probe": (None, [P]),
    "vlg_debug_set_gemm_bk": (None, [I]),
    "vlg_debug_set_gemm_run": (None, [I]),
}
CEPI_BIAS, CEPI_RESID, CEPI_PRELU, CEPI_DPRELU, CEPI_ACCUM, CEPI_CIN4 = 1, 2, 4, 8, 16, 32
CONV_PRECISIONS = ("fp32", "bf16")


def conv_sym(name: str, precision: str) -> str:
    if precision not in CONV_PRECISIONS:
        raise ValueError("conv precision must be one of %s, not %r" % (CONV_PRECISIONS, precision))
    if precision == "fp32":
        return name
    op = name.split("_")[2]
    pre = "vlg_conv3x3_" + op
    return pre + "_bf16" + name[len(pre):]

_lib = None


class HipError(RuntimeError):
    pass


def load() -> ctypes.CDLL:
    global _lib
    if _lib is not None:
        return _lib
    if not os.path.exists(LIB_PATH):
        raise HipError(
            "libvlg_hip.so not found at %s - run `python -c 'import __graft_entry__ as g; g.build()'` "
            "(or `make -C video-layout-generation_amd/csrc`); there is no CPU fallback" % LIB_PATH)
    import torch
    lib = ctypes.CDLL(LIB_PATH)
    for name, (res, args) in SIGNATURES.items():
        fn = getattr(lib, name)
        fn.restype = res
        fn.argtypes = args
    for name, (res, args) in DIAG_SIGNATURES.items():
        if hasattr(lib, name):
            fn = getattr(lib, name)
            fn.restype = res
            fn.argtypes = args
    _lib = lib
    return lib


def require_diag() -> ctypes.CDLL:
    lib = load()
    if not hasattr(lib, "vlg_debug_set_clock_probe"):
        raise HipError("this tool needs the diagnostic build: `make -C video-layout-generation_amd/csrc diag` and run with "
                       "VLG_HIP_LIB=<repo>/video-layout-generation_amd/libvlg_hip_diag.so (the product library has no debug switches)")
    return lib


_ERR = {1001: "VLG_ERR_SHAPE (unsupported or inconsistent shape)", 1002: "VLG_ERR_ALIGN (pointer / leading dimension not 16-byte aligned)"}


def check(code: int, what: str) -> None:
    if code != 0:
        raise HipError("%s failed: %s" % (what, _ERR.get(code, "hipError_t %d" % code)))


def ptr(t) -> int:
    return 0 if t is None else t.data_ptr()


tracer = None


def call(name: str, *args) -> None:
    cm = tracer(name, args) if tracer is not None else None
    if cm is None:
        check(getattr(load(), name)(*args), name)
        return
    with cm:
        check(getattr(load(), name)(*args), name)
```

Measured before the change: 5784.

## Fuse final layernorm, head linear, loss and their backward into one tail kernel

Adds one kernel that runs the final layernorm, the head projection, the layout loss and the backward through head and layernorm in a single pass. Each block writes per-block partial gradients for lnf_g, lnf_b, head_w and head_b into slabs, which are reduced into the flat gradient buffer. This replaces several launches and the round trips of the xf, out, dout and dh intermediates. The shared loss and row-IO code is moved into headers. It is enabled by default for fp32 when d is 128 or 256, and it adds a slab reduction step plus extra per-block work for the weight gradients.

```diff
diff --git a/include/vlg_hip.h b/include/vlg_hip.h
--- a/include/vlg_hip.h
+++ b/include/vlg_hip.h
@@ -112,6 +112,16 @@
                     const float* valid, float* dout, float* loss_out, float* scratch,
                     int B, int T, int N, int n_classes, float beta, float iou_eps,
                     float w_reg, float w_iou, float w_ce, void* stream);
+
+int     vlg_layout_tail_supported(int d, int n_classes);
+int     vlg_layout_tail_slabs(int64_t rows);
+int64_t vlg_layout_tail_slab_stride(int d);
+int     vlg_layout_tail_fwd_bwd(const float* x, const float* gamma, const float* beta, const float* head_w,
+                                const float* head_b, const int64_t* tgt_class, const float* tgt_box, const float* valid,
+                                float* out, int ld_out, float* dx, float* slabs, int64_t slab_stride,
+                                int64_t slab_capacity, float* loss_out, float* scratch, int B, int T, int N, int d,
+                                int n_classes, float ln_eps, float beta_sl1, float iou_eps, float w_reg, float w_iou,
+                                float w_ce, int max_blocks, void* stream);
 
 int vlg_attention_clip_fwd(const float* qkv, const float* valid, float* out, float* lse,
                            int64_t B, int T, int N, int d, void* stream);
diff --git a/video-layout-generation_amd/csrc/layernorm.hip b/video-layout-generation_amd/csrc/layernorm.hip
--- a/video-layout-generation_amd/csrc/layernorm.hip
+++ b/video-layout-generation_amd/csrc/layernorm.hip
@@ -1,40 +1,9 @@
 #include "common.h"
+#include "row_io.h"
 
 #define LN_BLOCK 256
 #define LN_WAVES (LN_BLOCK / 64)
 #define LN_BWD_MAX_BLOCKS 512
-
-template <int E, bool V4>
-struct RowIO {
-    template <typename EL>
-    __device__ static __forceinline__ void load(const EL* __restrict__ row, int lane, float (&v)[E]) {
-        if constexpr (V4) {
-#pragma unroll
-            for (int i = 0; i < E / 4; ++i) {
-                const float4 t = ld4(row + 4 * lane + 256 * i);
-                v[4 * i] = t.x; v[4 * i + 1] = t.y; v[4 * i + 2] = t.z; v[4 * i + 3] = t.w;
-            }
-        } else {
-#pragma unroll
-            for (int i = 0; i < E; ++i) v[i] = ld1(row + lane + 64 * i);
-        }
-    }
-    template <typename EL>
-    __device__ static __forceinline__ void store(EL* __restrict__ row, int lane, const float (&v)[E]) {
-        if constexpr (V4) {
-#pragma unroll
-            for (int i = 0; i < E / 4; ++i)
-                st4(row + 4 * lane + 256 * i, make_float4(v[4 * i], v[4 * i + 1], v[4 * i + 2], v[4 * i + 3]));
-        } else {
-#pragma unroll
-            for (int i = 0; i < E; ++i) st1(row + lane + 64 * i, v[i]);
-        }
-    }
-    __device__ static __forceinline__ int col(int lane, int j) {
-        if constexpr (V4) return 4 * lane + 256 * (j >> 2) + (j & 3);
-        else return lane + 64 * j;
-    }
-};
 
 #define LN_ROWS(E) ((E) <= 4 ? 4 : (E) <= 8 ? 2 : 1)
 
diff --git a/video-layout-generation_amd/csrc/loss.hip b/video-layout-generation_amd/csrc/loss.hip
--- a/video-layout-generation_amd/csrc/loss.hip
+++ b/video-layout-generation_amd/csrc/loss.hip
@@ -1,15 +1,8 @@
 #include "common.h"
+#include "loss_body.h"
 
-#define LOSS_BLOCK 256
 #define LOSS_TOK 128
-#define LOSS_ROWF 28
-#define LOSS_MAX_BLOCKS 1024
-#define NCLS 20
-#define NOUT (NCLS + 4)
-#define LOSS_F4 (NOUT / 4)
 #define LOSS_NV (LOSS_TOK * LOSS_F4 / LOSS_BLOCK)
-
-#define LOSS_SCRATCH (4 + 4 * LOSS_MAX_BLOCKS)
 
 __global__ __launch_bounds__(LOSS_BLOCK) void layout_loss_kernel(
     const float* __restrict__ out, int ld, const int64_t* __restrict__ tgt_class,
@@ -37,35 +30,13 @@
         int64_t cls = 0;
         float4 tb = f4_zero();
         if (mine) {
-            const int t = (int)(m % T);
-            const int64_t bn = m / T;
-            const int n = (int)(bn % N);
-            const int64_t b = bn / N;
-            const int64_t src = (b * T + t) * N + n;
+            const int64_t src = loss_src_index(m, T, N);
             w = valid[src];
             cls = tgt_class[src];
             tb = ld4(tgt_box + src * 4);
         }
         if (m0 == (int64_t)blockIdx.x * LOSS_TOK) {
-            float c = 0.f;
-            const int64_t n4 = M >> 2;
-            int64_t i = tid;
-            for (; i + 15 * LOSS_BLOCK < n4; i += 16 * LOSS_BLOCK) {
-                float4 v[16];
-#pragma unroll
-                for (int u = 0; u < 16; ++u) v[u] = ld4(valid + 4 * (i + u * LOSS_BLOCK));
-#pragma unroll
-                for (int u = 0; u < 16; ++u) c += (v[u].x + v[u].y) + (v[u].z + v[u].w);
-            }
-            for (; i < n4; i += LOSS_BLOCK) {
-                const float4 v = ld4(valid + 4 * i);
-                c += (v.x + v.y) + (v.z + v.w);
-            }
-            for (int64_t j = 4 * n4 + tid; j < M; j += LOSS_BLOCK) c += valid[j];
-            c = block_sum(c, red);
-            if (tid == 0) cnt_sh = 1.0f / fmaxf(c, 1.0f);
-            __syncthreads();
-            inv_cnt = cnt_sh;
+            inv_cnt = loss_inv_count(valid, M, tid, red, &cnt_sh);
         }
 #pragma unroll
         for (int i = 0; i < LOSS_NV; ++i) {
@@ -75,72 +46,7 @@
         __syncthreads();
         if (mine) {
             float* row = rows + tid * LOSS_ROWF;
-            float v[NOUT];
-#pragma unroll
-            for (int c = 0; c < LOSS_F4; ++c) {
-                const float4 q = ld4(row + 4 * c);
-                v[4 * c] = q.x; v[4 * c + 1] = q.y; v[4 * c + 2] = q.z; v[4 * c + 3] = q.w;
-            }
-            float g[NOUT];
-            cls = cls < 0 ? 0 : (cls >= NCLS ? NCLS - 1 : cls);
-            float mx = v[0];
-#pragma unroll
-            for (int c = 1; c < NCLS; ++c) mx = fmaxf(mx, v[c]);
-            float se = 0.f, vt = 0.f;
-#pragma unroll
-            for (int c = 0; c < NCLS; ++c) {
-                g[c] = expf(v[c] - mx);
-                se += g[c];
-                vt = (c == cls) ? v[c] : vt;
-            }
-            const float ce = logf(se) + mx - vt;
-            const float gs = w * inv_cnt * w_ce / se;
-#pragma unroll
-            for (int c = 0; c < NCLS; ++c) g[c] = g[c] * gs - ((c == cls) ? w * inv_cnt * w_ce : 0.f);
-            const float tg[4] = {tb.x, tb.y, tb.z, tb.w};
-            float p[4], dp[4];
-            float reg = 0.f;
-#pragma unroll
-            for (int k = 0; k < 4; ++k) {
-                p[k] = 1.0f / (1.0f + expf(-v[NCLS + k]));
-                const float df = p[k] - tg[k], ad = fabsf(df);
-                const bool quad = ad < beta;
-                reg += quad ? 0.5f * df * df / beta : ad - 0.5f * beta;
-                dp[k] = (quad ? df / beta : (df > 0.f ? 1.f : (df < 0.f ? -1.f : 0.f))) * (w_reg * 0.25f);
-            }
-            const float ax1 = p[0] - 0.5f * p[2], ax2 = p[0] + 0.5f * p[2];
-            const float ay1 = p[1] - 0.5f * p[3], ay2 = p[1] + 0.5f * p[3];
-            const float bx1 = tg[0] - 0.5f * tg[2], bx2 = tg[0] + 0.5f * tg[2];
-            const float by1 = tg[1] - 0.5f * tg[3], by2 = tg[1] + 0.5f * tg[3];
-            const float iw_raw = fminf(ax2, bx2) - fmaxf(ax1, bx1);
-            const float ih_raw = fminf(ay2, by2) - fmaxf(ay1, by1);
-            const float iw = fmaxf(iw_raw, 0.f), ih = fmaxf(ih_raw, 0.f);
-            const float inter = iw * ih;
-            const float uni = p[2] * p[3] + tg[2] * tg[3] - inter;
-            const float den = uni + iou_eps;
-            const float iou = inter / den;
-            const float di_dinter = (den + inter) / (den * den);
-            const float di_darea = -inter / (den * den);
-            const float x2s = (ax2 < bx2) ? 1.f : (ax2 == bx2 ? 0.5f : 0.f);
-            const float x1s = (ax1 > bx1) ? 1.f : (ax1 == bx1 ? 0.5f : 0.f);
-            const float y2s = (ay2 < by2) ? 1.f : (ay2 == by2 ? 0.5f : 0.f);
-            const float y1s = (ay1 > by1) ? 1.f : (ay1 == by1 ? 0.5f : 0.f);
-            const float diw = (iw_raw >= 0.f) ? ih * di_dinter : 0.f;
-            const float dih = (ih_raw >= 0.f) ? iw * di_dinter : 0.f;
-            float di[4];
-            di[0] = diw * (x2s - x1s);
-            di[1] = dih * (y2s - y1s);
-            di[2] = diw * 0.5f * (x2s + x1s) + di_darea * p[3];
-            di[3] = dih * 0.5f * (y2s + y1s) + di_darea * p[2];
-#pragma unroll
-            for (int k = 0; k < 4; ++k)
-                g[NCLS + k] = (dp[k] - w_iou * di[k]) * p[k] * (1.f - p[k]) * w * inv_cnt;
-#pragma unroll
-            for (int c = 0; c < LOSS_F4; ++c)
-                st4(row + 4 * c, make_float4(g[4 * c], g[4 * c + 1], g[4 * c + 2], g[4 * c + 3]));
-            s_reg += w * reg * 0.25f;
-            s_iou += w * (1.f - iou);
-            s_ce += w * ce;
+            loss_token(row, cls, tb, w, inv_cnt, beta, iou_eps, w_reg, w_iou, w_ce, s_reg, s_iou, s_ce);
         }
         __syncthreads();
 #pragma unroll
@@ -150,32 +56,7 @@
         }
         __syncthreads();
     }
-    s_reg = block_sum(s_reg, red);
-    s_iou = block_sum(s_iou, red);
-    s_ce = block_sum(s_ce, red);
-    if (tid == 0) {
-        float* part = scratch + 4 + 4 * blockIdx.x;
-        part[0] = s_reg * inv_cnt; part[1] = s_iou * inv_cnt; part[2] = s_ce * inv_cnt; part[3] = 0.f;
-        __threadfence();
-        int* ticket = reinterpret_cast<int*>(scratch) + 1;
-        const int drawn = atomicAdd(ticket, 1);
-        last_sh = (drawn == (int)gridDim.x - 1) ? 1 : 0;
-    }
-    __syncthreads();
-    if (last_sh && tid < 64) {
-        __threadfence();
-        float a = 0.f, b = 0.f, c = 0.f;
-        for (int i = tid; i < (int)gridDim.x; i += 64) {
-            const float4 q = ld4(scratch + 4 + 4 * i);
-            a += q.x; b += q.y; c += q.z;
-        }
-        a = wave_sum(a); b = wave_sum(b); c = wave_sum(c);
-        if (tid == 0) {
-            loss_out[0] = w_reg * a + w_iou * b + w_ce * c;
-            loss_out[1] = a; loss_out[2] = b; loss_out[3] = c;
-            *(reinterpret_cast<int*>(scratch) + 1) = 0;
-        }
-    }
+    loss_finish(s_reg, s_iou, s_ce, inv_cnt, scratch, loss_out, red, &last_sh, w_reg, w_iou, w_ce);
 }
 
 extern "C" int vlg_layout_loss_scratch(void) { return LOSS_SCRATCH; }
diff --git a/video-layout-generation_amd/csrc/loss_body.h b/video-layout-generation_amd/csrc/loss_body.h
--- /dev/null
+++ b/video-layout-generation_amd/csrc/loss_body.h
@@ -0,0 +1,144 @@
+#pragma once
+#include "common.h"
+
+#define LOSS_BLOCK 256
+#define LOSS_ROWF 28
+#define LOSS_MAX_BLOCKS 1024
+#define NCLS 20
+#define NOUT (NCLS + 4)
+#define LOSS_F4 (NOUT / 4)
+
+#define LOSS_SCRATCH (4 + 4 * LOSS_MAX_BLOCKS)
+
+__device__ __forceinline__ int64_t loss_src_index(int64_t m, int T, int N) {
+    const int t = (int)(m % T);
+    const int64_t bn = m / T;
+    const int n = (int)(bn % N);
+    const int64_t b = bn / N;
+    return (b * T + t) * N + n;
+}
+
+__device__ __forceinline__ float loss_inv_count(const float* __restrict__ valid, int64_t M, int tid, float* red, float* cnt_sh) {
+    float c = 0.f;
+    const int64_t n4 = M >> 2;
+    int64_t i = tid;
+    for (; i + 15 * LOSS_BLOCK < n4; i += 16 * LOSS_BLOCK) {
+        float4 v[16];
+#pragma unroll
+        for (int u = 0; u < 16; ++u) v[u] = ld4(valid + 4 * (i + u * LOSS_BLOCK));
+#pragma unroll
+        for (int u = 0; u < 16; ++u) c += (v[u].x + v[u].y) + (v[u].z + v[u].w);
+    }
+    for (; i < n4; i += LOSS_BLOCK) {
+        const float4 v = ld4(valid + 4 * i);
+        c += (v.x + v.y) + (v.z + v.w);
+    }
+    for (int64_t j = 4 * n4 + tid; j < M; j += LOSS_BLOCK) c += valid[j];
+    c = block_sum(c, red);
+    if (tid == 0) *cnt_sh = 1.0f / fmaxf(c, 1.0f);
+    __syncthreads();
+    return *cnt_sh;
+}
+
+__device__ __forceinline__ void loss_token(float* row, int64_t cls, float4 tb, float w, float inv_cnt, float beta,
+                                           float iou_eps, float w_reg, float w_iou, float w_ce, float& s_reg,
+                                           float& s_iou, float& s_ce) {
+    float v[NOUT];
+#pragma unroll
+    for (int c = 0; c < LOSS_F4; ++c) {
+        const float4 q = ld4(row + 4 * c);
+        v[4 * c] = q.x; v[4 * c + 1] = q.y; v[4 * c + 2] = q.z; v[4 * c + 3] = q.w;
+    }
+    float g[NOUT];
+    cls = cls < 0 ? 0 : (cls >= NCLS ? NCLS - 1 : cls);
+    float mx = v[0];
+#pragma unroll
+    for (int c = 1; c < NCLS; ++c) mx = fmaxf(mx, v[c]);
+    float se = 0.f, vt = 0.f;
+#pragma unroll
+    for (int c = 0; c < NCLS; ++c) {
+        g[c] = expf(v[c] - mx);
+        se += g[c];
+        vt = (c == cls) ? v[c] : vt;
+    }
+    const float ce = logf(se) + mx - vt;
+    const float gs = w * inv_cnt * w_ce / se;
+#pragma unroll
+    for (int c = 0; c < NCLS; ++c) g[c] = g[c] * gs - ((c == cls) ? w * inv_cnt * w_ce : 0.f);
+    const float tg[4] = {tb.x, tb.y, tb.z, tb.w};
+    float p[4], dp[4];
+    float reg = 0.f;
+#pragma unroll
+    for (int k = 0; k < 4; ++k) {
+        p[k] = 1.0f / (1.0f + expf(-v[NCLS + k]));
+        const float df = p[k] - tg[k], ad = fabsf(df);
+        const bool quad = ad < beta;
+        reg += quad ? 0.5f * df * df / beta : ad - 0.5f * beta;
+        dp[k] = (quad ? df / beta : (df > 0.f ? 1.f : (df < 0.f ? -1.f : 0.f))) * (w_reg * 0.25f);
+    }
+    const float ax1 = p[0] - 0.5f * p[2], ax2 = p[0] + 0.5f * p[2];
+    const float ay1 = p[1] - 0.5f * p[3], ay2 = p[1] + 0.5f * p[3];
+    const float bx1 = tg[0] - 0.5f * tg[2], bx2 = tg[0] + 0.5f * tg[2];
+    const float by1 = tg[1] - 0.5f * tg[3], by2 = tg[1] + 0.5f * tg[3];
+    const float iw_raw = fminf(ax2, bx2) - fmaxf(ax1, bx1);
+    const float ih_raw = fminf(ay2, by2) - fmaxf(ay1, by1);
+    const float iw = fmaxf(iw_raw, 0.f), ih = fmaxf(ih_raw, 0.f);
+    const float inter = iw * ih;
+    const float uni = p[2] * p[3] + tg[2] * tg[3] - inter;
+    const float den = uni + iou_eps;
+    const float iou = inter / den;
+    const float di_dinter = (den + inter) / (den * den);
+    const float di_darea = -inter / (den * den);
+    const float x2s = (ax2 < bx2) ? 1.f : (ax2 == bx2 ? 0.5f : 0.f);
+    const float x1s = (ax1 > bx1) ? 1.f : (ax1 == bx1 ? 0.5f : 0.f);
+    const float y2s = (ay2 < by2) ? 1.f : (ay2 == by2 ? 0.5f : 0.f);
+    const float y1s = (ay1 > by1) ? 1.f : (ay1 == by1 ? 0.5f : 0.f);
+    const float diw = (iw_raw >= 0.f) ? ih * di_dinter : 0.f;
+    const float dih = (ih_raw >= 0.f) ? iw * di_dinter : 0.f;
+    float di[4];
+    di[0] = diw * (x2s - x1s);
+    di[1] = dih * (y2s - y1s);
+    di[2] = diw * 0.5f * (x2s + x1s) + di_darea * p[3];
+    di[3] = dih * 0.5f * (y2s + y1s) + di_darea * p[2];
+#pragma unroll
+    for (int k = 0; k < 4; ++k)
+        g[NCLS + k] = (dp[k] - w_iou * di[k]) * p[k] * (1.f - p[k]) * w * inv_cnt;
+#pragma unroll
+    for (int c = 0; c < LOSS_F4; ++c)
+        st4(row + 4 * c, make_float4(g[4 * c], g[4 * c + 1], g[4 * c + 2], g[4 * c + 3]));
+    s_reg += w * reg * 0.25f;
+    s_iou += w * (1.f - iou);
+    s_ce += w * ce;
+}
+
+__device__ __forceinline__ void loss_finish(float s_reg, float s_iou, float s_ce, float inv_cnt, float* __restrict__ scratch,
+                                            float* __restrict__ loss_out, float* red, int* last_sh, float w_reg,
+                                            float w_iou, float w_ce) {
+    const int tid = threadIdx.x;
+    s_reg = block_sum(s_reg, red);
+    s_iou = block_sum(s_iou, red);
+    s_ce = block_sum(s_ce, red);
+    if (tid == 0) {
+        float* part = scratch + 4 + 4 * blockIdx.x;
+        part[0] = s_reg * inv_cnt; part[1] = s_iou * inv_cnt; part[2] = s_ce * inv_cnt; part[3] = 0.f;
+        __threadfence();
+        int* ticket = reinterpret_cast<int*>(scratch) + 1;
+        const int drawn = atomicAdd(ticket, 1);
+        *last_sh = (drawn == (int)gridDim.x - 1) ? 1 : 0;
+    }
+    __syncthreads();
+    if (*last_sh && tid < 64) {
+        __threadfence();
+        float a = 0.f, b = 0.f, c = 0.f;
+        for (int i = tid; i < (int)gridDim.x; i += 64) {
+            const float4 q = ld4(scratch + 4 + 4 * i);
+            a += q.x; b += q.y; c += q.z;
+        }
+        a = wave_sum(a); b = wave_sum(b); c = wave_sum(c);
+        if (tid == 0) {
+            loss_out[0] = w_reg * a + w_iou * b + w_ce * c;
+            loss_out[1] = a; loss_out[2] = b; loss_out[3] = c;
+            *(reinterpret_cast<int*>(scratch) + 1) = 0;
+        }
+    }
+}
diff --git a/video-layout-generation_amd/csrc/row_io.h b/video-layout-generation_amd/csrc/row_io.h
--- /dev/null
+++ b/video-layout-generation_amd/csrc/row_io.h
@@ -0,0 +1,34 @@
+#pragma once
+#include "common.h"
+
+template <int E, bool V4>
+struct RowIO {
+    template <typename EL>
+    __device__ static __forceinline__ void load(const EL* __restrict__ row, int lane, float (&v)[E]) {
+        if constexpr (V4) {
+#pragma unroll
+            for (int i = 0; i < E / 4; ++i) {
+                const float4 t = ld4(row + 4 * lane + 256 * i);
+                v[4 * i] = t.x; v[4 * i + 1] = t.y; v[4 * i + 2] = t.z; v[4 * i + 3] = t.w;
+            }
+        } else {
+#pragma unroll
+            for (int i = 0; i < E; ++i) v[i] = ld1(row + lane + 64 * i);
+        }
+    }
+    template <typename EL>
+    __device__ static __forceinline__ void store(EL* __restrict__ row, int lane, const float (&v)[E]) {
+        if constexpr (V4) {
+#pragma unroll
+            for (int i = 0; i < E / 4; ++i)
+                st4(row + 4 * lane + 256 * i, make_float4(v[4 * i], v[4 * i + 1], v[4 * i + 2], v[4 * i + 3]));
+        } else {
+#pragma unroll
+            for (int i = 0; i < E; ++i) st1(row + lane + 64 * i, v[i]);
+        }
+    }
+    __device__ static __forceinline__ int col(int lane, int j) {
+        if constexpr (V4) return 4 * lane + 256 * (j >> 2) + (j & 3);
+        else return lane + 64 * j;
+    }
+};
diff --git a/video-layout-generation_amd/csrc/tail.hip b/video-layout-generation_amd/csrc/tail.hip
--- /dev/null
+++ b/video-layout-generation_amd/csrc/tail.hip
@@ -0,0 +1,302 @@
+#include "common.h"
+#include "loss_body.h"
+#include "row_io.h"
+
+typedef float tail_acc __attribute__((ext_vector_type(16)));
+
+#define TAIL_ROWS 64
+#define TAIL_MAX_BLOCKS 512
+
+__device__ __forceinline__ int tail_acc_row(int q, int h) { return (q & 3) + 8 * (q >> 2) + 4 * h; }
+
+template <int D>
+__global__ __launch_bounds__(LOSS_BLOCK) void layout_tail_kernel(
+    const float* __restrict__ x, const float* __restrict__ gamma, const float* __restrict__ beta,
+    const float* __restrict__ head_w, const float* __restrict__ head_b, const int64_t* __restrict__ tgt_class,
+    const float* __restrict__ tgt_box, const float* __restrict__ valid, float* __restrict__ out, int ldo,
+    float* __restrict__ dx, float* __restrict__ slabs, int64_t slab_stride, float* __restrict__ scratch,
+    float* __restrict__ loss_out, int B, int T, int N, float eps, float sl1_beta, float iou_eps, float w_reg, float w_iou,
+    float w_ce) {
+    constexpr int E = D / 64;
+    constexpr bool V4 = D % 256 == 0;
+    constexpr int LDX = D + 4;
+    constexpr int NT = D / 32;
+    constexpr int NH = NT / 2;
+    constexpr int NW = NT / 4;
+    constexpr int RB = E <= 4 ? 4 : 2;
+    static_assert(D % 128 == 0 && TAIL_ROWS * LOSS_F4 <= 2 * LOSS_BLOCK && 8 * D <= TAIL_ROWS * LDX, "tile plan");
+    __shared__ __attribute__((aligned(16))) float xt[TAIL_ROWS * LDX];
+    __shared__ __attribute__((aligned(16))) float ot[TAIL_ROWS * LOSS_ROWF];
+    __shared__ float rs_sh[TAIL_ROWS];
+    __shared__ float sums[2][TAIL_ROWS][2];
+    __shared__ float red[LOSS_BLOCK / 64];
+    __shared__ float cnt_sh;
+    __shared__ int last_sh;
+    const int64_t M = (int64_t)B * T * N;
+    const int tid = threadIdx.x;
+#define TAIL_LANE_IDS(t)                                                                                         \
+    const int lane = (t) & 63, w = (t) >> 6, l31 = lane & 31, h = lane >> 5, rt = w & 1, hf = w >> 1;            \
+    const int jc = l31 < NOUT ? l31 : NOUT - 1;                                                                  \
+    const bool jreal = l31 < NOUT
+
+    const float inv_cnt = loss_inv_count(valid, M, tid, red, &cnt_sh);
+
+    tail_acc wacc[NW];
+#pragma unroll
+    for (int i = 0; i < NW; ++i)
+#pragma unroll
+        for (int q = 0; q < 16; ++q) wacc[i][q] = 0.f;
+    float dg[NH], dbt[NH], dbias = 0.f;
+#pragma unroll
+    for (int i = 0; i < NH; ++i) { dg[i] = 0.f; dbt[i] = 0.f; }
+    float s_reg = 0.f, s_iou = 0.f, s_ce = 0.f;
+
+    for (int64_t m0 = (int64_t)blockIdx.x * TAIL_ROWS; m0 < M; m0 += (int64_t)gridDim.x * TAIL_ROWS) {
+        int opaque = 0, tid_o = tid;
+        asm volatile("" : "+s"(opaque), "+v"(tid_o));
+        const float* __restrict__ gam = gamma + opaque;
+        const float* __restrict__ bet = beta + opaque;
+        const float* __restrict__ hw = head_w + opaque;
+        TAIL_LANE_IDS(tid_o);
+        const bool mine = tid < TAIL_ROWS && m0 + tid < M;
+        float tw = 0.f;
+        int64_t cls = 0;
+        float4 tb = f4_zero();
+        if (mine) {
+            const int64_t src = loss_src_index(m0 + tid, T, N);
+            tw = valid[src];
+            cls = tgt_class[src];
+            tb = ld4(tgt_box + src * 4);
+        }
+#pragma unroll 1
+        for (int rb = 0; rb < TAIL_ROWS / 4; rb += RB) {
+            float v[RB][E];
+#pragma unroll
+            for (int i = 0; i < RB; ++i) {
+                const int64_t r = m0 + w * 16 + rb + i;
+                RowIO<E, V4>::load(x + (r < M ? r : M - 1) * D, lane, v[i]);
+            }
+#pragma unroll
+            for (int i = 0; i < RB; ++i) {
+                const int r = w * 16 + rb + i;
+                const bool live = m0 + r < M;
+                float s = 0.f;
+#pragma unroll
+                for (int j = 0; j < E; ++j) s += v[i][j];
+                const float mu = wave_sum(s) * (1.0f / D);
+                float q = 0.f;
+#pragma unroll
+                for (int j = 0; j < E; ++j) { const float t = v[i][j] - mu; q += t * t; }
+                const float rs = 1.0f / sqrtf(wave_sum(q) * (1.0f / D) + eps);
+#pragma unroll
+                for (int j = 0; j < E; ++j) v[i][j] = live ? (v[i][j] - mu) * rs : 0.f;
+                RowIO<E, V4>::store(xt + r * LDX, lane, v[i]);
+                if (lane == 0) rs_sh[r] = live ? rs : 0.f;
+            }
+        }
+        __syncthreads();
+        {
+            tail_acc acc;
+#pragma unroll
+            for (int q = 0; q < 16; ++q) acc[q] = 0.f;
+            const int k0 = hf * (D / 2) + 4 * h;
+            const float* arow = xt + (rt * 32 + l31) * LDX + k0;
+            const float* wrow = hw + jc * D + k0;
+#pragma unroll 2
+            for (int s = 0; s < D / 16; ++s) {
+                const float4 a = ld4(arow + 8 * s), g4 = ld4(gam + k0 + 8 * s), b4 = ld4(bet + k0 + 8 * s);
+                float4 w4 = ld4(wrow + 8 * s);
+                if (!jreal) w4 = f4_zero();
+                acc = __builtin_amdgcn_mfma_f32_32x32x2f32(a.x * g4.x + b4.x, w4.x, acc, 0, 0, 0);
+                acc = __builtin_amdgcn_mfma_f32_32x32x2f32(a.y * g4.y + b4.y, w4.y, acc, 0, 0, 0);
+                acc = __builtin_amdgcn_mfma_f32_32x32x2f32(a.z * g4.z + b4.z, w4.z, acc, 0, 0, 0);
+                acc = __builtin_amdgcn_mfma_f32_32x32x2f32(a.w * g4.w + b4.w, w4.w, acc, 0, 0, 0);
+            }
+            float* ocol = ot + (rt * 32 + 4 * h) * LOSS_ROWF + l31;
+            if (hf == 1 && jreal) {
+#pragma unroll
+                for (int q = 0; q < 16; ++q) ocol[tail_acc_row(q, 0) * LOSS_ROWF] = acc[q];
+            }
+            __syncthreads();
+            if (hf == 0 && jreal) {
+                const float bias_j = head_b[jc + opaque];
+#pragma unroll
+                for (int q = 0; q < 16; ++q) {
+                    float* o = ocol + tail_acc_row(q, 0) * LOSS_ROWF;
+                    *o = (acc[q] + *o) + bias_j;
+                }
+            }
+            __syncthreads();
+        }
+        for (int f = tid; f < TAIL_ROWS * LOSS_F4; f += LOSS_BLOCK) {
+            const int tok = f / LOSS_F4, c = f - tok * LOSS_F4;
+            if (m0 + tok < M) st4(out + (m0 + tok) * ldo + 4 * c, ld4(ot + tok * LOSS_ROWF + 4 * c));
+        }
+        __syncthreads();
+        if (tid < TAIL_ROWS) {
+            float* row = ot + tid * LOSS_ROWF;
+            if (mine) loss_token(row, cls, tb, tw, inv_cnt, sl1_beta, iou_eps, w_reg, w_iou, w_ce, s_reg, s_iou, s_ce);
+            else {
+#pragma unroll
+                for (int c = 0; c < LOSS_F4; ++c) st4(row + 4 * c, f4_zero());
+            }
+        }
+        __syncthreads();
+        float gam_w[NW], bet_w[NW];
+#pragma unroll
+        for (int i = 0; i < NW; ++i) { gam_w[i] = gam[(w * NW + i) * 32 + l31]; bet_w[i] = bet[(w * NW + i) * 32 + l31]; }
+#pragma unroll 8
+        for (int kk = 0; kk < TAIL_ROWS / 2; ++kk) {
+            const int r = 2 * kk + h;
+            float a = ot[r * LOSS_ROWF + jc];
+            a = jreal ? a : 0.f;
+            if (w == 0) dbias += a;
+#pragma unroll
+            for (int i = 0; i < NW; ++i) {
+                const float b = xt[r * LDX + (w * NW + i) * 32 + l31] * gam_w[i] + bet_w[i];
+                wacc[i] = __builtin_amdgcn_mfma_f32_32x32x2f32(a, b, wacc[i], 0, 0, 0);
+            }
+        }
+        tail_acc dacc[NH];
+#pragma unroll
+        for (int i = 0; i < NH; ++i)
+#pragma unroll
+            for (int q = 0; q < 16; ++q) dacc[i][q] = 0.f;
+#pragma unroll
+        for (int s = 0; s < NOUT / 8; ++s) {
+            const float4 a4 = ld4(ot + (rt * 32 + l31) * LOSS_ROWF + 8 * s + 4 * h);
+            const float a[4] = {a4.x, a4.y, a4.z, a4.w};
+#pragma unroll
+            for (int i = 0; i < NH; ++i)
+#pragma unroll
+                for (int j = 0; j < 4; ++j)
+                    dacc[i] = __builtin_amdgcn_mfma_f32_32x32x2f32(a[j], hw[(8 * s + 4 * h + j) * D + (hf * NH + i) * 32 + l31],
+                                                                   dacc[i], 0, 0, 0);
+        }
+        __syncthreads();
+        {
+            float s1[16], s2[16];
+#pragma unroll
+            for (int q = 0; q < 16; ++q) { s1[q] = 0.f; s2[q] = 0.f; }
+            float* xcol = xt + (rt * 32 + 4 * h) * LDX + hf * NH * 32 + l31;
+            float gam_h[NH];
+#pragma unroll
+            for (int i = 0; i < NH; ++i) gam_h[i] = gam[(hf * NH + i) * 32 + l31];
+#pragma unroll
+            for (int i = 0; i < NH; ++i) {
+#pragma unroll
+                for (int q = 0; q < 16; ++q) {
+                    const float xh = xcol[tail_acc_row(q, 0) * LDX + 32 * i];
+                    const float gy = dacc[i][q];
+                    const float a = gy * gam_h[i];
+                    dg[i] += gy * xh;
+                    dbt[i] += gy;
+                    s1[q] += a;
+                    s2[q] += a * xh;
+                    dacc[i][q] = a;
+                }
+                __builtin_amdgcn_sched_barrier(0);
+            }
+#pragma unroll
+            for (int q = 0; q < 16; ++q) { s1[q] = group_sum<32>(s1[q]); s2[q] = group_sum<32>(s2[q]); }
+            if (l31 == 0) {
+#pragma unroll
+                for (int q = 0; q < 16; ++q) {
+                    const int r = rt * 32 + tail_acc_row(q, h);
+                    sums[hf][r][0] = s1[q];
+                    sums[hf][r][1] = s2[q];
+                }
+            }
+            __syncthreads();
+#pragma unroll
+            for (int q = 0; q < 16; ++q) {
+                const int r = rt * 32 + tail_acc_row(q, h);
+                const float t1 = (sums[0][r][0] + sums[1][r][0]) * (1.0f / D);
+                const float t2 = (sums[0][r][1] + sums[1][r][1]) * (1.0f / D);
+                const float rs = rs_sh[r];
+#pragma unroll
+                for (int i = 0; i < NH; ++i) {
+                    float* p = xcol + tail_acc_row(q, 0) * LDX + 32 * i;
+                    *p = rs * (dacc[i][q] - t1 - *p * t2);
+                }
+                if ((q & 3) == 3) __builtin_amdgcn_sched_barrier(0);
+            }
+        }
+        __syncthreads();
+        for (int f = tid; f < TAIL_ROWS * (D / 4); f += LOSS_BLOCK) {
+            const int r = f / (D / 4), c = f - r * (D / 4);
+            if (m0 + r < M) st4(dx + (m0 + r) * D + 4 * c, ld4(xt + r * LDX + 4 * c));
+        }
+        __syncthreads();
+    }
+
+    float* slab = slabs + (int64_t)blockIdx.x * slab_stride;
+    const int lane = tid & 63, w = tid >> 6, l31 = lane & 31, h = lane >> 5, rt = w & 1, hf = w >> 1;
+    {
+        float* rg = xt;
+        const int slot = rt * 2 + h;
+#pragma unroll
+        for (int i = 0; i < NH; ++i) {
+            const int c = (hf * NH + i) * 32 + l31;
+            rg[slot * 2 * D + c] = dg[i];
+            rg[slot * 2 * D + D + c] = dbt[i];
+        }
+        __syncthreads();
+        for (int c = tid; c < 2 * D; c += LOSS_BLOCK)
+            slab[c] = ((rg[c] + rg[2 * D + c]) + rg[4 * D + c]) + rg[6 * D + c];
+    }
+#pragma unroll
+    for (int i = 0; i < NW; ++i)
+#pragma unroll
+        for (int q = 0; q < 16; ++q) {
+            const int j = tail_acc_row(q, h);
+            if (j < NOUT) slab[2 * D + j * D + (w * NW + i) * 32 + l31] = wacc[i][q];
+        }
+    dbias += __shfl_xor(dbias, 32);
+    if (w == 0 && lane < NOUT) slab[(2 + NOUT) * D + lane] = dbias;
+
+    loss_finish(s_reg, s_iou, s_ce, inv_cnt, scratch, loss_out, red, &last_sh, w_reg, w_iou, w_ce);
+}
+
+static bool tail_supported(int d, int n_classes) {
+    if (VLG_TUNE("VLG_TAIL_FUSED", 1) == 0) return false;
+    return n_classes == NCLS && (d == 128 || d == 256);
+}
+static int tail_blocks(int64_t rows, int max_blocks) {
+    int64_t b = (rows + TAIL_ROWS - 1) / TAIL_ROWS;
+    const int64_t cap = max_blocks > 0 && max_blocks < TAIL_MAX_BLOCKS ? max_blocks : TAIL_MAX_BLOCKS;
+    return (int)(b > cap ? cap : (b < 1 ? 1 : b));
+}
+
+extern "C" int vlg_layout_tail_supported(int d, int n_classes) { return tail_supported(d, n_classes) ? 1 : 0; }
+extern "C" int vlg_layout_tail_slabs(int64_t rows) { return tail_blocks(rows, 0); }
+extern "C" int64_t vlg_layout_tail_slab_stride(int d) { return (int64_t)(2 + NOUT) * d + NOUT; }
+
+extern "C" int vlg_layout_tail_fwd_bwd(const float* x, const float* gamma, const float* beta, const float* head_w,
+                                       const float* head_b, const int64_t* tgt_class, const float* tgt_box,
+                                       const float* valid, float* out, int ld_out, float* dx, float* slabs,
+                                       int64_t slab_stride, int64_t slab_capacity, float* loss_out, float* scratch, int B,
+                                       int T, int N, int d, int n_classes, float ln_eps, float beta_sl1, float iou_eps,
+                                       float w_reg, float w_iou, float w_ce, int max_blocks, void* stream) {
+    if (!tail_supported(d, n_classes) || B < 1 || T < 1 || N < 1 || ld_out < NOUT || (ld_out & 3) || !(beta_sl1 > 0.f) ||
+        max_blocks < 0)
+        return VLG_ERR_SHAPE;
+    const int64_t M = (int64_t)B * T * N;
+    const int blocks = tail_blocks(M, max_blocks);
+    if (slab_stride < vlg_layout_tail_slab_stride(d) || slab_capacity < (int64_t)blocks * slab_stride) return VLG_ERR_SHAPE;
+    if (!vlg_aligned16(x) || !vlg_aligned16(gamma) || !vlg_aligned16(beta) || !vlg_aligned16(head_w) || !vlg_aligned16(out) ||
+        !vlg_aligned16(dx) || !vlg_aligned16(tgt_box) || !vlg_aligned16(valid) || !head_b || !tgt_class || !slabs ||
+        !loss_out || !scratch || !vlg_aligned16(scratch))
+        return VLG_ERR_ALIGN;
+    hipStream_t s = (hipStream_t)stream;
+#define CALL(DD)                                                                                                            \
+    hipLaunchKernelGGL((layout_tail_kernel<DD>), dim3((unsigned)blocks), dim3(LOSS_BLOCK), 0, s, x, gamma, beta, head_w,    \
+                       head_b, tgt_class, tgt_box, valid, out, ld_out, dx, slabs, slab_stride, scratch, loss_out, B, T, N, \
+                       ln_eps, beta_sl1, iou_eps, w_reg, w_iou, w_ce)
+    switch (d) {
+        case 128: CALL(128); break;
+        default: CALL(256); break;
+    }
+#undef CALL
+    return vlg_last_error();
+}
diff --git a/video-layout-generation_amd/vlg/engine.py b/video-layout-generation_amd/vlg/engine.py
--- a/video-layout-generation_amd/vlg/engine.py
+++ b/video-layout-generation_amd/vlg/engine.py
@@ -37,7 +37,8 @@
 class LayoutEngine:
 
     def __init__(self, cfg: LayoutConfig, device: torch.device, seed: int = 1024,
-                 lr: float = ADAM_LR, beta1: float = ADAM_BETA1, precision: str = "fp32", padded_slots: bool = True):
+                 lr: float = ADAM_LR, beta1: float = ADAM_BETA1, precision: str = "fp32", padded_slots: bool = True,
+                 fused_tail: Optional[bool] = None):
         cfg.validate()
         if precision not in ("fp32", "bf16", "bf16_mfma", "fp32x3"):
             raise ValueError("precision must be fp32, fp32x3, bf16 or bf16_mfma")
@@ -54,6 +55,10 @@
         if device.type != "cuda":
             raise hip.HipError("LayoutEngine needs a HIP device (got %s); there is no CPU path" % device)
         self.cfg, self.device = cfg, device
+        can_fuse = precision == "fp32" and bool(hip.load().vlg_layout_tail_supported(cfg.d, cfg.n_classes))
+        if fused_tail and not can_fuse:
+            raise ValueError("fused_tail=True needs precision fp32 and a shape the library's tail kernel supports")
+        self.fused_tail = can_fuse if fused_tail is None else bool(fused_tail)
         self.lr, self.beta1 = float(lr), float(beta1)
         self.layout, self.n_params = param_layout(cfg)
         f32 = dict(dtype=torch.float32, device=device)
@@ -153,6 +158,11 @@
         self.du = torch.empty(M, ff, **act)
         self.dqkv = torch.empty(M, 3 * d, **act)
         self.loss_scratch = torch.zeros(lib.vlg_layout_loss_scratch(), **f32)
+        if self.fused_tail:
+            self._tail_stride = int(lib.vlg_layout_tail_slab_stride(d))
+            if self.n_params - self.layout["lnf_g"][0] != self._tail_stride:
+                raise RuntimeError("flat-gradient tail does not match the tail kernel's slab layout")
+            self.tail_slabs = torch.empty(lib.vlg_layout_tail_slabs(M) * self._tail_stride, **f32)
         if cfg.attention == "clip":
             self.lse = torch.empty(L, cfg.n_heads * M, **f32)
             self.delta = torch.empty(cfg.n_heads * M, **f32)
@@ -375,6 +385,14 @@
             self._linear(self.gl[l], self.pw(pre + "ff2_w"), self.p(pre + "ff2_b"), self.x[l + 1], M, d, ff,
                          EPI_BIAS | EPI_RESID, aux_in=self.xmid[l])
         L = cfg.n_layers
+        if self.fused_tail:
+            self._timed("tail", 3 * 2.0 * M * d * 32, "vlg_layout_tail_fwd_bwd", ptr(self.x[L]), ptr(self.p("lnf_g")),
+                        ptr(self.p("lnf_b")), ptr(self.p("head_w")), ptr(self.p("head_b")), ptr(batch["tgt_class"]),
+                        ptr(batch["tgt_box"]), ptr(batch["valid"]), ptr(self.out), cfg.n_out, ptr(self.dx),
+                        ptr(self.tail_slabs), self._tail_stride, self.tail_slabs.numel(), ptr(self.loss_out),
+                        ptr(self.loss_scratch), B, T, N, d, cfg.n_classes, LN_EPS, SMOOTH_L1_BETA, IOU_EPS, LOSS_W_REG,
+                        LOSS_W_STRUCT, LOSS_W_CE, 0, s, nbytes=2.0 * 4 * M * d + 4.0 * M * cfg.n_out + (8 + 16 + 4) * M)
+            return self.loss_out
         self._ln_fwd(self.x[L], "lnf_g", self.xf, self.stats[2 * L], M)
         self._linear(self.xf, self.pw("head_w"), self.p("head_b"), self.out, M, cfg.n_out, d, EPI_BIAS)
         self._timed("loss", 0.0, "vlg_layout_loss", ptr(self.out), cfg.n_out, ptr(batch["tgt_class"]), ptr(batch["tgt_box"]),
@@ -421,9 +439,19 @@
 
         if self.group_reduce:
             self._gsel, self._goff, self._grows, self._pending = 0, 0, [], None
-        on_side(("dout",), lambda: self._wgrad(self.dout, self.xf, "head_w", M, cfg.n_out, d))
-        self._dgrad(self.dout, self.pw("head_w"), self.dh, M, cfg.n_out, d)
-        self._ln_bwd(self.dh, self.x[L], self.stats[2 * L], "lnf_g", None, self.dx, M)
+        if self.fused_tail:
+            n_slabs = hip.load().vlg_layout_tail_slabs(M)
+            off = self.layout["lnf_g"][0]
+            if self.group_reduce:
+                self._grows.append((self.tail_slabs.data_ptr(), self._tail_stride, n_slabs,
+                                    self.grads.data_ptr() + 4 * off, self._tail_stride))
+            else:
+                call("vlg_reduce_slabs", ptr(self.tail_slabs), self._tail_stride, n_slabs,
+                     self.grads.data_ptr() + 4 * off, self._tail_stride, s)
+        else:
+            on_side(("dout",), lambda: self._wgrad(self.dout, self.xf, "head_w", M, cfg.n_out, d))
+            self._dgrad(self.dout, self.pw("head_w"), self.dh, M, cfg.n_out, d)
+            self._ln_bwd(self.dh, self.x[L], self.stats[2 * L], "lnf_g", None, self.dx, M)
         ready = (lambda tag: (lambda: reducer.ready(tag))) if reducer is not None else (lambda tag: None)
         if reducer is not None or self.group_reduce:
             join()
diff --git a/video-layout-generation_amd/vlg/hip.py b/video-layout-generation_amd/vlg/hip.py
--- a/video-layout-generation_amd/vlg/hip.py
+++ b/video-layout-generation_amd/vlg/hip.py
@@ -43,6 +43,10 @@
     "vlg_attention_clip_bwd_bf16": (I, [P, P, P, P, P, P, P, L, I, I, I, P]),
     "vlg_layout_loss_scratch": (I, []),
     "vlg_layout_loss": (I, [P, I, P, P, P, P, P, P, I, I, I, I, F, F, F, F, F, P]),
+    "vlg_layout_tail_supported": (I, [I, I]),
+    "vlg_layout_tail_slabs": (I, [L]),
+    "vlg_layout_tail_slab_stride": (L, [I]),
+    "vlg_layout_tail_fwd_bwd": (I, [P, P, P, P, P, P, P, P, P, I, P, P, L, L, P, P, I, I, I, I, I, F, F, F, F, F, F, I, P]),
     "vlg_reduce_slabs": (I, [P, L, I, P, L, P]),
     "vlg_reduce_slabs_table": (I, [P, I, I, P]),
     "vlg_sum_partials_table": (I, [P, I, P]),
```

Result: no change. 5786, median of 5 (+0.0%).
